# Enigmatisms/cvx_proj

Measured on AMD Instinct MI355X. Metric: local homographies/sec + Mpix/sec warp, 4K pair 200x200 mesh, higher is better.
Workload: dtype f64; 1 GPU; C3: 3840x2160 pair, 2000 correspondences, 200x200 mesh, canvas 4009x2242; mode=pairs, variant=auto, launch=eager, parallelism=pairsx1

## Files before the change

### cvx_proj_amd/_native.py

```python
from __future__ import annotations

import ctypes as C
import os
import sys
from typing import NamedTuple

import numpy as np

_HERE = os.path.dirname(os.path.abspath(__file__))
LIB_PATH = os.environ.get("APAP_HIP_LIB") or os.path.join(_HERE, "libapap_hip.so")

OK, ERR_INVALID_ARG, ERR_NO_DEVICE, ERR_HIP, ERR_SINGULAR, ERR_INDEX, ERR_WORKSPACE = range(7)
ABI_VERSION = 6
PROF_NAMES = ("assemble", "eigen", "invert", "lut", "warp", "eq_hist", "eq_apply", "ransac", "spectral")
PROF_SLOTS = len(PROF_NAMES)
TABLE_STRIDE = 32
DENORM_DOUBLES = 36
VARIANT_AUTO, VARIANT_VALU, VARIANT_MFMA, VARIANT_MFMA4, VARIANT_MFMA4X2 = 0, 1, 2, 3, 4
EIGEN_AUTO, EIGEN_JACOBI, EIGEN_INVERSE_ITERATION = 0, 1, 2
OPT_SOLVER_VARIANT, OPT_EIGEN_SOLVER, OPT_CAREFUL, OPT_PROFILE, OPT_WANT_WAVES, OPT_WARP_ROWS, OPT_WEIGHT_CHUNK_KB, \
    OPT_FUSED_MAX_CELLS, OPT_WARP_FAST, OPT_OVERLAP_PCIE, OPT_PLAN_CELLS, OPT_MOMENTS, OPT_WEIGHTS_F32, \
    OPT_PLAN_SLOTS, OPT_WARP_SAMPLING = range(15)
SAMPLING_NEAREST, SAMPLING_BILINEAR = 0, 1
SAMPLINGS = {"nearest": SAMPLING_NEAREST, "bilinear": SAMPLING_BILINEAR}


class ApapError(RuntimeError):

    def __init__(self, code, message):
        super().__init__(f"[apap_hip error {code}] {message}")
        self.code = code


class ApapSingularError(ApapError, np.linalg.LinAlgError):
    """APAP_ERR_SINGULAR: ``numpy.linalg.inv`` of a cell raised LinAlgError("Singular matrix")
    (apap.py:165-166,203,252)."""


class ApapIndexError(ApapError, IndexError):
    """APAP_ERR_INDEX: ``np.where(i < mesh_h)[0][0]`` found no edge above a canvas index
    (apap.py:207,209)."""


class ApapValueError(ApapError, ValueError):
    """APAP_ERR_INVALID_ARG: what the reference's shape unpacking rejects with ValueError
    (apap.py:129-130,197,199)."""


_ERROR_CLASSES = {ERR_SINGULAR: ApapSingularError, ERR_INDEX: ApapIndexError, ERR_INVALID_ARG: ApapValueError}

STATUS_SINGULAR, STATUS_INDEX, STATUS_UNPREPARED = 1, 2, 4
STATUS_NO_CONVERGENCE = 8
STATUS_MODEL_DEGENERATE = 16
STATUS_MODEL_NO_CONVERGENCE = 32


def raise_for_status(word, who):
    if word & STATUS_SINGULAR:
        raise ApapSingularError(ERR_SINGULAR, f"{who}: Singular matrix")
    if word & STATUS_INDEX:
        raise ApapIndexError(ERR_INDEX, f"{who}: index 0 is out of bounds for axis 0 with size 0 (mesh edges do not cover the canvas)")
    if word & STATUS_UNPREPARED:
        raise ApapValueError(ERR_INVALID_ARG, f"{who}: the warp workspace holds no lookup tables for this mesh / canvas "
                                              "(APAP_WARP_GEOMETRY)")


_f32p = C.POINTER(C.c_float)
_f64p = C.POINTER(C.c_double)
_u8p = C.POINTER(C.c_uint8)
_i32p = C.POINTER(C.c_int)
_i64p = C.POINTER(C.c_longlong)
_vp = C.c_void_p

SIGNATURES = {
    "apap_last_error": (C.c_char_p, []),
    "apap_version": (C.c_char_p, []),
    "apap_abi_version": (C.c_int, []),
    "apap_device_count": (C.c_int, []),
    "apap_ctx_create": (C.c_void_p, []),
    "apap_ctx_destroy": (None, [_vp]),
    "apap_ctx_set_option": (C.c_int, [_vp, C.c_int, C.c_int]),
    "apap_ctx_get_option": (C.c_int, [_vp, C.c_int, _i32p]),
    "apap_ctx_profile_read": (C.c_int, [_vp, _f32p, _i32p]),
    "apap_host_prepare": (C.c_int, [_f32p, _f32p, C.c_int] + [_f32p] * 10),
    "apap_host_dlt_rows": (C.c_int, [_f32p, _f32p, C.c_int, _f32p]),
    "apap_host_prepare_pts": (C.c_int, [_vp, C.c_int, _vp, C.c_int, C.c_int] + [_f32p] * 6 + [_f64p] * 4),
    "apap_host_dlt_rows_pts": (C.c_int, [_f64p, _f64p, C.c_int, C.c_int, _f32p]),
    "apap_host_build_table_rows": (C.c_int, [_f64p, _f32p, C.c_int, _f64p]),
    "apap_host_build_table": (C.c_int, [_f32p, _f32p, _f32p, C.c_int, _f64p]),
    "apap_host_build_table24": (C.c_int, [_f64p, _f32p, C.c_int, _f64p]),
    "apap_host_build_denorm": (C.c_int, [_f32p, _f32p, _f32p, _f32p, _f64p]),
    "apap_local_homography": (C.c_int, [_vp, _f32p, _f32p, C.c_int, _f64p, C.c_int, C.c_int, C.c_double,
                                        C.c_double, _f32p, _f64p, C.c_int]),
    "apap_local_weights": (C.c_int, [_vp, _f32p, C.c_int, _f64p, C.c_int, C.c_double, C.c_double, _f64p, C.c_int]),
    "apap_local_homography_pts": (C.c_int, [_vp, _vp, C.c_int, _vp, C.c_int, C.c_int, _f64p, C.c_int, C.c_int, C.c_double,
                                            C.c_double, _f32p, _f64p, C.c_int]),
    "apap_local_weights_pts": (C.c_int, [_vp, _vp, C.c_int, C.c_int, _f64p, C.c_int, C.c_double, C.c_double, _f64p, C.c_int]),
    "apap_local_warp": (C.c_int, [_vp, _u8p, C.c_int, C.c_int, _f32p, C.c_int, C.c_int, _f64p, C.c_int, _f64p,
                                  C.c_int, C.c_int, C.c_int, C.c_int, C.c_int, _u8p, _f32p, C.c_int]),
    "apap_local_warp_f64": (C.c_int, [_vp, _u8p, C.c_int, C.c_int, _f64p, C.c_int, C.c_int, _f64p, C.c_int, _f64p,
                                      C.c_int, C.c_int, C.c_int, C.c_int, C.c_int, _u8p, _f64p, C.c_int]),
    "apap_local_stitch": (C.c_int, [_vp, _u8p, C.c_int, C.c_int, _u8p, C.c_int, C.c_int, _f32p, C.c_int, C.c_int, _f64p,
                                    C.c_int, _f64p, C.c_int, C.c_int, C.c_int, C.c_int, C.c_int, _u8p, _f32p, C.c_int]),
    "apap_warp_coords": (C.c_int, [_vp, _f32p, C.c_int, C.c_int, _f64p, C.c_int, _f64p, C.c_int, C.c_int, C.c_int,
                                   C.c_int, C.c_int, _f64p, C.c_int]),
    "apap_invert_normalize_flatten": (C.c_int, [_vp, _f32p, C.c_int, _f64p, C.c_int]),
    "apap_uniform_blend": (C.c_int, [_vp, _u8p, _u8p, C.c_int, C.c_int, _u8p, C.c_int]),
    "apap_solve_workspace_bytes": (C.c_size_t, [_vp, C.c_int, C.c_int]),
    "apap_solve_device": (C.c_int, [_vp, _vp, C.c_int, _vp, C.c_int, C.c_double, C.c_double, _vp, _vp, _vp,
                                    C.c_size_t, _vp]),
    "apap_solve_batch_workspace_bytes": (C.c_size_t, [_vp, C.c_int, C.c_int, C.c_int]),
    "apap_solve_batch_device": (C.c_int, [_vp, _vp, C.c_int, _vp, C.c_longlong, C.c_int, C.c_double, C.c_double, _vp, _vp,
                                          C.c_int, _vp, C.c_size_t, _vp]),
    "apap_solve_warp_batch_device": (C.c_int, [_vp, _vp, C.c_int, _vp, C.c_longlong, C.c_double, C.c_double, _vp, _vp, C.c_int, _vp,
                                               C.c_size_t, C.c_int, C.c_int, _vp, C.c_int, _vp, C.c_int, C.c_int, C.c_int, C.c_int,
                                               C.c_int, _vp, C.c_size_t, _vp, _vp]),
    "apap_weights_device": (C.c_int, [_vp, _vp, C.c_int, _vp, C.c_int, C.c_double, C.c_double, _vp, _vp]),
    "apap_warp_workspace_bytes": (C.c_size_t, [C.c_int, C.c_int, C.c_int, C.c_int]),
    "apap_warp_device": (C.c_int, [_vp, _vp, C.c_int, C.c_int, _vp, C.c_int, C.c_int, _vp, C.c_int, _vp, C.c_int,
                                   C.c_int, C.c_int, C.c_int, C.c_int, _vp, _vp, _vp, C.c_size_t, _vp, _vp]),
    "apap_warp_f64_device": (C.c_int, [_vp, _vp, C.c_int, C.c_int, _vp, C.c_int, C.c_int, _vp, C.c_int, _vp, C.c_int,
                                       C.c_int, C.c_int, C.c_int, C.c_int, _vp, _vp, _vp, C.c_size_t, _vp, _vp]),
    "apap_warp_rows_device": (C.c_int, [_vp, _vp, C.c_int, C.c_int, _vp, C.c_int, C.c_int, _vp, C.c_int, _vp, C.c_int,
                                        C.c_int, C.c_int, C.c_int, C.c_int, C.c_int, C.c_int, _vp, _vp, C.c_size_t, _vp,
                                        _vp]),
    "apap_warp_batch_workspace_bytes": (C.c_size_t, [C.c_int, C.c_int, C.c_int, C.c_int, C.c_int]),
    "apap_warp_batch_device": (C.c_int, [_vp, _vp, C.c_longlong, C.c_int, C.c_int, _vp, C.c_longlong, C.c_int, C.c_int, _vp, C.c_int,
                                         C.c_int, _vp, C.c_int, _vp, C.c_int, C.c_int, C.c_int, C.c_int, C.c_int, C.c_int, C.c_int,
                                         _vp, C.c_longlong, _vp, C.c_int, C.c_int, _vp, C.c_size_t, _vp, _vp]),
    "apap_stitch_device": (C.c_int, [_vp, _vp, C.c_int, C.c_int, _vp, C.c_int, C.c_int, _vp, C.c_int, C.c_int, _vp, C.c_int,
                                     _vp, C.c_int, C.c_int, C.c_int, C.c_int, C.c_int, _vp, _vp, _vp, C.c_size_t, _vp, _vp]),
    "apap_warp_coords_device": (C.c_int, [_vp, _vp, C.c_int, C.c_int, _vp, C.c_int, _vp, C.c_int, C.c_int, C.c_int,
                                          C.c_int, C.c_int, _vp, _vp, C.c_size_t, _vp, _vp]),
    "apap_flatten_device": (C.c_int, [_vp, _vp, C.c_int, _vp, _vp, _vp]),
    "apap_blend_device": (C.c_int, [_vp, _vp, _vp, C.c_int, C.c_int, _vp, _vp]),
    "apap_equalize_hist": (C.c_int, [_vp, _u8p, C.c_int, C.c_int, C.c_int, _u8p, C.c_int]),
    "apap_equalize_workspace_bytes": (C.c_size_t, [C.c_int]),
    "apap_equalize_hist_device": (C.c_int, [_vp, _vp, C.c_int, C.c_int, C.c_int, _vp, _vp, C.c_size_t, _vp]),
    "apap_find_homography_ransac": (C.c_int, [_vp, _f32p, _f32p, C.c_int, C.c_double, C.c_int, C.c_ulonglong, _f64p, _u8p,
                                              _i32p, C.c_int]),
    "apap_ransac_workspace_bytes": (C.c_size_t, [C.c_int, C.c_int]),
    "apap_ransac_device": (C.c_int, [_vp, _vp, _vp, C.c_int, C.c_double, C.c_int, C.c_ulonglong, _vp, _vp, _vp, _vp,
                                     C.c_size_t, _vp]),
    "apap_spectral_weights": (C.c_int, [_vp, _f32p, _f32p, _f32p, _f32p, C.c_int, _f64p, _f64p, _f32p, _f32p, _f64p, _f32p,
                                        _f32p, _f64p, C.c_int]),
    "apap_spectral_workspace_bytes": (C.c_size_t, [C.c_int]),
    "apap_spectral_device": (C.c_int, [_vp, _vp, _vp, _vp, _vp, C.c_int, _vp, _f64p, _vp, _vp, _vp, _vp, _vp, _vp, _vp, _vp,
                                       C.c_size_t, _vp]),
    "apap_spectral_affinity": (C.c_int, [_vp, _f32p, _f32p, _f32p, _f32p, C.c_int, _f64p, _f64p, _f64p, C.c_int]),
    "apap_model_solve": (C.c_int, [_vp, _f32p, _f32p, _f32p, C.c_int, _f64p, _f32p, _f64p, C.c_int]),
    "apap_model_workspace_bytes": (C.c_size_t, [C.c_int]),
    "apap_model_solve_device": (C.c_int, [_vp, _vp, _vp, _vp, C.c_int, _f64p, _vp, _vp, _vp, _vp, C.c_size_t, _vp]),
    "apap_spectral_em": (C.c_int, [_vp, _f32p, _f32p, _f32p, _f32p, C.c_int, _f64p, _f64p, _f64p, C.c_int, _f32p, _f32p, _f64p,
                                   _f64p, _f32p, _f32p, _f64p, C.c_int]),
    "apap_spectral_em_device": (C.c_int, [_vp, _vp, _vp, _vp, _vp, C.c_int, _vp, _f64p, _f64p, C.c_int, _vp, _vp, _vp, _vp, _vp, _vp,
                                          _vp, _vp, _vp, C.c_size_t, _vp]),
    "apap_spectral_em_batch_workspace_bytes": (C.c_size_t, [_i32p, C.c_int, _i32p, C.c_int]),
    "apap_spectral_em_batch_device": (C.c_int, [_vp, _vp, _vp, _vp, _vp, _vp, _vp, _i32p, C.c_int, _i32p, _f64p, _f64p, C.c_int,
                                                C.c_int, _vp, _vp, _vp, _vp, _vp, _vp, _vp, _vp, C.c_size_t, _vp]),
    "apap_spectral_em_batch": (C.c_int, [_vp, _f32p, _f32p, _f32p, _f32p, _f64p, _f32p, _i32p, C.c_int, _i32p, _f64p, _f64p,
                                         C.c_int, C.c_int, _f32p, _f64p, _f64p, _f32p, _f32p, _f64p, _i32p, C.c_int]),
    "apap_local_model_workspace_bytes": (C.c_size_t, [C.c_int, C.c_int]),
    "apap_local_model_solve_device": (C.c_int, [_vp, _vp, _vp, _vp, C.c_int, _vp, C.c_int, C.c_double, C.c_double, _f64p, _vp, _vp,
                                                _vp, _vp, C.c_size_t, _vp]),
    "apap_local_model_solve": (C.c_int, [_vp, _f32p, _f32p, _f32p, C.c_int, _f64p, C.c_int, C.c_double, C.c_double, _f64p, _f32p,
                                         _f64p, _i32p, C.c_int]),
    "apap_match_workspace_bytes": (C.c_size_t, [C.c_int, C.c_int]),
    "apap_match_descriptors": (C.c_int, [_vp, _f32p, C.c_int, _f32p, C.c_int, _i32p, _f32p, _i32p, _f32p, C.c_int]),
    "apap_match_descriptors_device": (C.c_int, [_vp, _vp, C.c_int, _vp, C.c_int, _vp, _vp, _vp, _vp, _vp, C.c_size_t, _vp]),
    "apap_match_batch_workspace_bytes": (C.c_size_t, [_i32p, _i32p, C.c_int]),
    "apap_match_descriptors_batch": (C.c_int, [_vp, _f32p, _f32p, _i32p, _i32p, C.c_int, _i32p, _f32p, _i32p, _f32p, C.c_int]),
    "apap_match_descriptors_batch_device": (C.c_int, [_vp, _vp, _vp, _i32p, _i32p, C.c_int, _vp, _vp, _vp, _vp, _vp, C.c_size_t,
                                                      _vp]),
    "apap_sift_window": (C.c_int, [_f32p]),
    "apap_sift_taps": (C.c_int, [_f32p]),
    "apap_sift_workspace_bytes": (C.c_size_t, [C.c_int]),
    "apap_sift_describe": (C.c_int, [_vp, _u8p, C.c_int, C.c_int, C.c_int, _f32p, C.c_int, _f32p, C.c_int]),
    "apap_sift_describe_device": (C.c_int, [_vp, _vp, C.c_int, C.c_int, C.c_int, _vp, C.c_int, _vp, _vp, C.c_size_t, _vp]),
    "apap_sift_describe_batch": (C.c_int, [_vp, C.POINTER(C.c_void_p), _i32p, _i32p, _i32p, C.c_int, _f32p, _i32p, _f32p, C.c_int]),
    "apap_sift_describe_batch_device": (C.c_int, [_vp, C.POINTER(C.c_void_p), _i32p, _i32p, _i32p, C.c_int, _vp, _i32p, _vp, _vp,
                                                  C.c_size_t, _vp]),
    "apap_corner_workspace_bytes": (C.c_size_t, [_i32p, _i32p, C.c_int, C.c_int]),
    "apap_corner_detect": (C.c_int, [_vp, _u8p, C.c_int, C.c_int, C.c_int, C.c_int, C.c_int, C.c_int, _f32p, _i64p, _i32p, C.c_int]),
    "apap_corner_detect_device": (C.c_int, [_vp, _vp, C.c_int, C.c_int, C.c_int, C.c_int, C.c_int, C.c_int, _vp, _vp, _vp, _vp,
                                            C.c_size_t, _vp]),
    "apap_corner_detect_batch": (C.c_int, [_vp, C.POINTER(C.c_void_p), _i32p, _i32p, _i32p, C.c_int, C.c_int, C.c_int, C.c_int, _f32p,
                                           _i64p, _i32p, C.c_int]),
    "apap_corner_detect_batch_device": (C.c_int, [_vp, C.POINTER(C.c_void_p), _i32p, _i32p, _i32p, C.c_int, C.c_int, C.c_int, C.c_int,
                                                  _vp, _vp, _vp, _vp, C.c_size_t, _vp]),
    "apap_image_warp_bounds": (C.c_int, [C.c_int, C.c_int, C.c_int, C.c_int, _f64p, _i32p]),
    "apap_image_warp_workspace_bytes": (C.c_size_t, [C.c_int]),
    "apap_image_warp": (C.c_int, [_vp, _u8p, C.c_int, C.c_int, _u8p, C.c_int, C.c_int, _f64p, C.c_int, C.c_int, C.c_int, C.c_int,
                                  C.c_int, _u8p, C.c_int]),
    "apap_image_warp_device": (C.c_int, [_vp, _vp, C.c_int, C.c_int, _vp, C.c_int, C.c_int, _f64p, C.c_int, C.c_int, C.c_int, C.c_int,
                                         C.c_int, _vp, _vp, C.c_size_t, _vp, _vp]),
    "apap_image_warp_batch": (C.c_int, [_vp, C.POINTER(C.c_void_p), _i32p, _i32p, C.POINTER(C.c_void_p), _i32p, _i32p, _f64p, _i32p,
                                        _i32p, _i32p, _i32p, _i32p, C.c_int, _u8p, _i64p, C.c_int]),
    "apap_image_warp_batch_device": (C.c_int, [_vp, C.POINTER(C.c_void_p), _i32p, _i32p, C.POINTER(C.c_void_p), _i32p, _i32p, _f64p,
                                               _i32p, _i32p, _i32p, _i32p, _i32p, C.c_int, _vp, _i64p, _vp, C.c_size_t, _vp, _vp]),
    "apap_panorama_bounds": (C.c_int, [C.c_int, C.c_int, _i32p, _i32p, _i32p, _i32p, C.c_int, _i32p]),
    "apap_panorama_workspace_bytes": (C.c_size_t, [_i32p, _i32p, _i32p, _i32p, C.c_int]),
    "apap_panorama_mean_of": (C.c_uint, [C.c_uint, C.c_uint]),
    "apap_panorama": (C.c_int, [_vp, _u8p, C.c_int, C.c_int, C.POINTER(C.c_void_p), _i32p, _i32p, C.POINTER(C.c_void_p), _i32p, _i32p,
                                C.POINTER(C.c_void_p), _i32p, C.POINTER(C.c_void_p), _i32p, _i32p, _i32p, _i32p, _i32p, C.c_int, C.c_int,
                                _u8p, _i32p, C.c_int]),
    "apap_panorama_device": (C.c_int, [_vp, _vp, C.c_int, C.c_int, C.POINTER(C.c_void_p), _i32p, _i32p, C.POINTER(C.c_void_p), _i32p,
                                       _i32p, C.POINTER(C.c_void_p), _i32p, C.POINTER(C.c_void_p), _i32p, _i32p, _i32p, _i32p, _i32p,
                                       C.c_int, C.c_int, _vp, _vp, C.c_size_t, _vp, _vp]),
    "apap_panorama_ramp_weight": (C.c_int, [C.c_int, C.c_int, C.c_int, C.c_int, C.c_int]),
    "apap_panorama_ramp_quotients": (None, [C.POINTER(C.c_uint), C.POINTER(C.c_uint), C.c_int, C.POINTER(C.c_uint)]),
}
SIGNATURES["apap_panorama_ramp"] = SIGNATURES["apap_panorama"]
SIGNATURES["apap_panorama_ramp_device"] = SIGNATURES["apap_panorama_device"]
_u64p = C.POINTER(C.c_ulonglong)
_PANO_GEOMETRY = SIGNATURES["apap_panorama"][1][:19]
_PANO_GEOMETRY_DEVICE = SIGNATURES["apap_panorama_device"][1][:19]
SIGNATURES.update({
    "apap_panorama_gain_solve": (C.c_int, [_u64p, _u64p, C.c_int, C.c_double, C.c_double, _f64p, _i32p, _i32p]),
    "apap_panorama_gain_apply": (C.c_int, [_u8p, C.c_int, C.c_int, _u8p]),
    "apap_panorama_gain_stats": (C.c_int, _PANO_GEOMETRY + [C.c_int, _u64p, _u64p, _i32p, C.c_int]),
    "apap_panorama_gain_stats_device": (C.c_int, _PANO_GEOMETRY_DEVICE + [C.c_int, _vp, _vp, _vp, C.c_size_t, _vp, _vp]),
    "apap_panorama_gain": (C.c_int, _PANO_GEOMETRY + [C.c_int, C.c_int, _i32p, _u8p, _i32p, C.c_int]),
    "apap_panorama_gain_device": (C.c_int, _PANO_GEOMETRY_DEVICE + [C.c_int, C.c_int, _i32p, _vp, _vp, C.c_size_t, _vp, _vp]),
    "apap_panorama_auto_gain": (C.c_int, _PANO_GEOMETRY + [C.c_int, C.c_int, C.c_int, C.c_double, C.c_double, _u8p, _u64p, _u64p, _f64p,
                                                           _i32p, _i32p, _i32p, C.c_int]),
    "apap_panorama_auto_gain_device": (C.c_int, _PANO_GEOMETRY_DEVICE + [C.c_int, C.c_int, C.c_int, C.c_double, C.c_double, _vp, _vp, _vp,
                                                                         _vp, _vp, _vp, _vp, C.c_size_t, _vp, _vp]),
})
SIGNATURES.update({
    "apap_box_blur": (C.c_int, [_vp, _u8p, C.c_int, C.c_int, C.c_int, _u8p, C.c_int]),
    "apap_box_blur_device": (C.c_int, [_vp, _vp, C.c_int, C.c_int, C.c_int, _vp, _vp]),
    "apap_panorama_band_workspace_bytes": (C.c_size_t, [C.c_int, C.c_int, _i32p, _i32p, _i32p, _i32p, _i32p, _i32p, C.c_int, C.c_int]),
    "apap_panorama_band": (C.c_int, _PANO_GEOMETRY + [C.c_int, C.c_int, _i32p, _u8p, _i32p, C.c_int]),
    "apap_panorama_band_device": (C.c_int, _PANO_GEOMETRY_DEVICE + [C.c_int, C.c_int, _i32p, _vp, _vp, C.c_size_t, _vp, _vp]),
})

_lib = None
_torch_at_load = False


def lib():
    global _lib, _torch_at_load
    if _lib is None:
        if not os.path.exists(LIB_PATH):
            raise ApapError(ERR_NO_DEVICE, f"{LIB_PATH} not built; run `python -c 'import __graft_entry__ as g; "
                                           "g.build()'` or `make -C cvx_proj_amd/csrc`")
        if "torch" not in sys.modules and os.environ.get("APAP_HIP_PRELOAD_TORCH", "0") == "1":
            try:
                import torch
            except ImportError:
                pass
        _torch_at_load = "torch" in sys.modules
        handle = C.CDLL(LIB_PATH)
        got = handle.apap_abi_version() if hasattr(handle, "apap_abi_version") else 1
        if got != ABI_VERSION:
            raise ApapError(ERR_INVALID_ARG, f"{LIB_PATH} is ABI generation {got}, this binding needs {ABI_VERSION}: rebuild "
                                             "it (make -C cvx_proj_amd/csrc)")
        for name, (res, args) in SIGNATURES.items():
            fn = getattr(handle, name)
            fn.restype = res
            fn.argtypes = args
        _lib = handle
    return _lib


def check(code):
    if code != OK:
        raise _ERROR_CLASSES.get(code, ApapError)(code, lib().apap_last_error().decode("utf-8", "replace"))


class Context:

    def __init__(self, **options):
        self._h = lib().apap_ctx_create()
        if not self._h:
            raise ApapError(ERR_HIP, "apap_ctx_create failed")
        for k, v in options.items():
            self.set(k, v)

    _NAMES = {"variant": OPT_SOLVER_VARIANT, "eigen": OPT_EIGEN_SOLVER, "careful": OPT_CAREFUL, "profile": OPT_PROFILE,
              "want_waves": OPT_WANT_WAVES, "warp_rows": OPT_WARP_ROWS, "weight_chunk_kb": OPT_WEIGHT_CHUNK_KB,
              "fused_max_cells": OPT_FUSED_MAX_CELLS, "warp_fast": OPT_WARP_FAST, "overlap_pcie": OPT_OVERLAP_PCIE,
              "plan_cells": OPT_PLAN_CELLS, "moments": OPT_MOMENTS, "weights_f32": OPT_WEIGHTS_F32,
              "plan_slots": OPT_PLAN_SLOTS, "warp_sampling": OPT_WARP_SAMPLING}

    def set(self, name, value):
        check(lib().apap_ctx_set_option(self._h, self._NAMES[name], int(value)))
        return self

    def get(self, name):
        v = C.c_int(0)
        check(lib().apap_ctx_get_option(self._h, self._NAMES[name], C.byref(v)))
        return v.value

    def profile_read(self):
        ms = (C.c_float * PROF_SLOTS)()
        cnt = (C.c_int * PROF_SLOTS)()
        check(lib().apap_ctx_profile_read(self._h, ms, cnt))
        return {k: (ms[i], cnt[i]) for i, k in enumerate(PROF_NAMES)}

    @property
    def handle(self):
        return self._h

    def close(self):
        if self._h:
            lib().apap_ctx_destroy(self._h)
            self._h = None

    def __del__(self):
        try:
            self.close()
        except Exception:
            pass


def _h(ctx):
    if ctx is None:
        return None
    return C.c_void_p(ctx.handle if isinstance(ctx, Context) else ctx)


def last_error():
    return lib().apap_last_error().decode("utf-8", "replace")


def sampling_value(sampling, who="local_warp"):
    if sampling is None:
        return None
    if not isinstance(sampling, str) or sampling not in SAMPLINGS:
        raise ValueError(f"{who}: sampling must be None, 'nearest' or 'bilinear'; got {sampling!r}")
    return SAMPLINGS[sampling]


class sampling_scope:

    def __init__(self, ctx, sampling, who="local_warp"):
        self._value = sampling_value(sampling, who)
        self._ctx, self._own, self._before = ctx, None, None

    def __enter__(self):
        if self._value is None:
            return self._ctx
        if self._ctx is None:
            self._own = self._ctx = Context()
        before = C.c_int(0)
        check(lib().apap_ctx_get_option(_h(self._ctx), OPT_WARP_SAMPLING, C.byref(before)))
        self._before = before.value
        check(lib().apap_ctx_set_option(_h(self._ctx), OPT_WARP_SAMPLING, self._value))
        return self._ctx

    def __exit__(self, *exc):
        if self._before is not None:
            lib().apap_ctx_set_option(_h(self._ctx), OPT_WARP_SAMPLING, self._before)
        if self._own is not None:
            self._own.close()
        return False


def _ptr(a, ctype):
    return a.ctypes.data_as(C.POINTER(ctype)) if a is not None else None


def as_f32(a, shape_tail=None):
    a = np.ascontiguousarray(a, dtype=np.float32)
    if shape_tail is not None and tuple(a.shape[-len(shape_tail):]) != tuple(shape_tail):
        raise ValueError(f"expected trailing shape {shape_tail}, got {a.shape}")
    return a


def as_points(a):
    a = np.asarray(a)
    a = np.ascontiguousarray(a, dtype=np.float32 if a.dtype == np.float32 else np.float64)
    if a.shape[-1:] != (2,):
        raise ValueError(f"expected trailing shape (2,), got {a.shape}")
    return a, int(a.dtype == np.float64)


def _vptr(a):
    return a.ctypes.data_as(C.c_void_p)


def _ip(a):
    return a.ctypes.data_as(_i32p)


def _dp(a):
    return a.ctypes.data_as(_f64p)


def _addrs(addresses):
    return (C.c_void_p * len(addresses))(*addresses)


def _i32(values):
    return np.array(values, dtype=np.int32)


def _offsets(lengths, name, one, many, rows, max_count, max_rows):
    lengths = [int(x) for x in lengths]
    if not 1 <= len(lengths) <= max_count:
        raise ValueError(f"{name}: {len(lengths)} {many} (1 .. {max_count})")
    if any(not 1 <= x <= max_rows for x in lengths):
        raise ValueError(f"{name}: {one} holds 1 .. 2^{max_rows.bit_length() - 1} {rows}; got {lengths}")
    if sum(lengths) > np.iinfo(np.int32).max:
        raise ValueError(f"{name}: {sum(lengths)} {rows} in all exceed the int32 offsets")
    off = np.zeros(len(lengths) + 1, np.int32)
    off[1:] = np.cumsum(lengths)
    return off


def _image_table(got):
    return (_addrs([a.ctypes.data for a, _ in got]), _i32([a.shape[0] for a, _ in got]), _i32([a.shape[1] for a, _ in got]),
            _i32([c for _, c in got]))


def host_prepare(src, dst):
    src, s64 = as_points(src)
    dst, d64 = as_points(dst)
    if src.shape != dst.shape or src.ndim != 2:
        raise ValueError(f"src/dst must both be (n, 2); got {src.shape} and {dst.shape}")
    n = src.shape[0]
    out = {k: np.empty((3, 3), np.float32) for k in ("N1", "N2", "C1", "C2", "iC2", "iN2")}
    if not s64 and not d64:
        out.update({k: np.empty((n, 2), np.float32) for k in ("nf1", "nf2", "cf1", "cf2")})
        check(lib().apap_host_prepare(_ptr(src, C.c_float), _ptr(dst, C.c_float), n,
                                      *[_ptr(out[k], C.c_float) for k in
                                        ("N1", "N2", "C1", "C2", "iC2", "iN2", "nf1", "nf2", "cf1", "cf2")]))
        return out
    wide = {k: np.empty((n, 2), np.float64) for k in ("nf1", "nf2", "cf1", "cf2")}
    check(lib().apap_host_prepare_pts(_vptr(src), s64, _vptr(dst), d64, n,
                                      *[_ptr(out[k], C.c_float) for k in ("N1", "N2", "C1", "C2", "iC2", "iN2")],
                                      *[_ptr(wide[k], C.c_double) for k in ("nf1", "nf2", "cf1", "cf2")]))
    for k, is64 in (("nf1", s64), ("cf1", s64), ("nf2", d64), ("cf2", d64)):
        out[k] = wide[k] if is64 else wide[k].astype(np.float32)
    return out


def host_dlt_rows(cf1, cf2):
    cf1, a64 = as_points(cf1)
    cf2, b64 = as_points(cf2)
    n = cf1.shape[0]
    aa = np.empty((2 * n, 9), np.float32)
    if not a64 and not b64:
        check(lib().apap_host_dlt_rows(_ptr(cf1, C.c_float), _ptr(cf2, C.c_float), n, _ptr(aa, C.c_float)))
    else:
# ... 909 lines not shown
```

### cvx_proj_amd/csrc/apap_internal.h

```cpp
#pragma once
#include <cstddef>
#include <cstdint>

#include <mutex>
#include <vector>

#include "../../include/apap_hip.h"

namespace apap {

struct ProfSpan {
    int slot;
    void *a, *b;
};

struct DevSlot {
    void *ptr = nullptr;
    size_t cap = 0;
    int dev = -1;
};
enum { S_TABLE, S_VERT, S_DENORM, S_H, S_WORK, S_W, S_IMG, S_OUT, S_MESHW, S_MESHH, S_HINV, S_STATUS, S_AUX, S_COUNT };

}

struct apap_ctx {
    int opt[APAP_OPT_COUNT] = {APAP_VARIANT_AUTO, APAP_EIGEN_AUTO, 1, 0, 4096, 1, 1 << 20, 4096, 1, 0, 0, 30, 0, 0, APAP_SAMPLING_NEAREST};
    std::vector<apap::ProfSpan> spans;
    apap::DevSlot slots[apap::S_COUNT];
    std::mutex mu;
    void *streams[3] = {nullptr, nullptr, nullptr};
    std::vector<void *> events;
    void *pinned = nullptr;
    size_t pinned_cap = 0;
    int pipe_dev = -1;
    int k1_slots[3] = {0, 0, 0};
    int k1_slots_dev = -1;
};

namespace apap {

int opt(const apap_ctx *ctx, int which);

int fail(int code, const char *fmt, ...) __attribute__((format(printf, 2, 3)));

int hip_fail(int hip_error, const char *what);

struct ProfScope {
    ProfScope(apap_ctx *ctx, int slot, void *stream);
    ~ProfScope();
    ProfScope(const ProfScope &) = delete;
    ProfScope &operator=(const ProfScope &) = delete;

  private:
    apap_ctx *ctx_;
    void *stream_, *a_, *b_;
    int slot_;
    bool on_;
};

bool inv3_f64(const double in[9], double out[9]);
bool inv3_f32(const float in[9], float out[9]);

struct SolvePlan {
    int variant;
    int cells_pad;
    int cell_tiles;
    int splits;
    int pts_per_split;
    size_t moment_bytes;
};
SolvePlan plan_solve(int n, int cells, int variant, int batch, int want_waves, int plan_cells = 0, int moments = 30);
int plan_pairs(int cell_tiles, int splits, int batch, int slots);

constexpr int kWarpSetup = APAP_WARP_GEOMETRY | APAP_WARP_CELLS;
constexpr int kWarpRows = APAP_WARP_GATHER;
int warp_phase(apap_ctx *ctx, const uint8_t *d_img, int img_h, int img_w, const uint8_t *d_center, int center_h, int center_w,
               const float *d_Hfwd, int mesh_rows, int mesh_cols, const double *d_mesh_w, int n_w, const double *d_mesh_h,
               int n_h, int final_w, int final_h, int off_x, int off_y, uint8_t *d_out_band, float *d_Hinv_out, void *d_work,
               size_t work_bytes, int *d_status, void *stream, int row_begin, int row_count, int phase, int **d_src_rows);

struct WarpTables {
    const double *hinv_pad;
    const int *lut;
};
WarpTables warp_tables(void *d_work, int mesh_rows, int mesh_cols, int final_w, int final_h);

struct WarpGather {
    const uint8_t *img;
    const uint8_t *center;
    uint8_t *out;
    const double *hinv_pad;
    const int *lut;
    int *status;
    long long img_stride, center_stride, out_stride, hinv_stride;
    int img_h, img_w, center_h, center_w, mesh_rows, mesh_cols, final_w, final_h, off_x, off_y, row_begin, row_count;
};
int warp_bilinear_launch(apap_ctx *ctx, const WarpGather &g, int batch, void *stream);

int panorama_check(int center_h, int center_w, const int *img_h, const int *img_w, const int *mesh_rows, const int *mesh_cols,
                   const int *n_w, const int *n_h, const int *final_w, const int *final_h, const int *off_x, const int *off_y,
                   int n_layers, int mode, const int *ramp, int *bounds, const char *who);
int panorama_device(apap_ctx *ctx, const uint8_t *d_center, int center_h, int center_w, const uint8_t *const *d_imgs, const int *img_h,
                    const int *img_w, const float *const *d_Hfwd, const int *mesh_rows, const int *mesh_cols,
                    const double *const *d_mesh_w, const int *n_w, const double *const *d_mesh_h, const int *n_h, const int *final_w,
                    const int *final_h, const int *off_x, const int *off_y, int n_layers, int mode, const int *ramp, uint8_t *d_out,
                    void *d_work, size_t work_bytes, int *d_status, void *stream, const char *who);

struct PanoGeometry {
    const uint8_t *d_center;
    int center_h, center_w;
    const uint8_t *const *d_imgs;
    const int *img_h, *img_w;
    const float *const *d_Hfwd;
    const int *mesh_rows, *mesh_cols;
    const double *const *d_mesh_w;
    const int *n_w;
    const double *const *d_mesh_h;
    const int *n_h, *final_w, *final_h, *off_x, *off_y;
    int n_layers;
};
enum { kPanoPlain = 0, kPanoGain, kPanoStats, kPanoAuto };
struct PanoJob {
    int what = kPanoPlain;
    int mode = APAP_PANORAMA_MEAN;
    const int *ramp = nullptr;
    const int *band = nullptr;
    uint8_t *d_out = nullptr;
    const int *gain_q = nullptr;
    int step = 1;
    unsigned long long *d_N = nullptr, *d_S = nullptr;
    double sigma_n = 10.0, sigma_g = 0.1;
    double *d_g = nullptr;
    int *d_q = nullptr, *d_flag = nullptr;
};
int panorama_run(apap_ctx *ctx, const PanoGeometry &G, const PanoJob &J, void *d_work, size_t work_bytes, int *d_status, void *stream,
                 const char *who);
int panorama_band_check(int band, const char *who);
int box_blur_check(int h, int w, int radius, const char *who);
int panorama_gain_check(int n_views, const int *step, const int *gain_q, const double *sigma_n, const double *sigma_g, const char *who);
int panorama_gain_solve_host(const unsigned long long *N, const unsigned long long *S, int n_views, double sigma_n, double sigma_g,
                             double *g, int *q);

constexpr int kMoments = 30;

int spectral_run(apap_ctx *ctx, const float *d_src, const float *d_dst, const float *d_c, const float *d_o, int n,
                 const double *d_F, const double *params, const float *d_Hg, const float *d_mask, double *d_segment,
                 float *d_ransac, float *d_original, double *d_info, int *d_status, void *d_work, size_t work_bytes,
                 void *stream, int sync_each);
int spectral_em_run(apap_ctx *ctx, const float *d_src, const float *d_dst, const float *d_c_feats, const float *d_o_feats, int n,
                    const double *d_F, const double *spec_params, const double *model_params, int em_steps, const float *d_mask_in,
                    float *d_H, double *d_info, double *d_segment, float *d_ransac_mask, float *d_original_mask,
                    double *d_spec_info, int *d_status, void *d_work, size_t work_bytes, void *stream, int sync_each);
int spectral_em_batch_run(apap_ctx *ctx, const float *d_src, const float *d_dst, const float *d_c_feats, const float *d_o_feats,
                          const double *d_F, const float *d_mask_in, const int *pair_offset, int n_pairs, const int *pair_of,
                          const double *spec_params, const double *model_params, int n_problems, int em_steps, float *d_H,
                          double *d_info, double *d_segment, float *d_ransac_mask, float *d_original_mask, double *d_spec_info,
                          int *d_status, void *d_work, size_t work_bytes, void *stream, int sync_each);
int spectral_em_batch_check(const int *pair_offset, int n_pairs, const int *pair_of, const double *spec_params,
                            const double *model_params, int n_problems, int em_steps, const char *who);
int local_model_check(int n, int cells, double gamma, double sigma, const double *params, const char *who);
int match_check(const int *q_offset, const int *t_offset, int n_pairs, const char *who);
inline size_t up256(size_t bytes) { return (bytes + 255) / 256 * 256; }

constexpr int kImageMinSide = 7, kImageMaxSide = 32768, kMaxImages = 65535;
inline int image_sides_check(int m, int h, int w, const char *who) {
    if (h < kImageMinSide || h > kImageMaxSide || w < kImageMinSide || w > kImageMaxSide)
        return fail(APAP_ERR_INVALID_ARG, "%s: image %d is %d x %d (sides %d .. %d)", who, m, h, w, kImageMinSide, kImageMaxSide);
    return APAP_OK;
}
inline int image_channels_check(int m, int c, const char *who) {
    if (c != 1 && c != 3) return fail(APAP_ERR_INVALID_ARG, "%s: image %d has %d channels (1 = grey or 3 = BGR)", who, m, c);
    return APAP_OK;
}
int sift_check(const int *heights, const int *widths, const int *channels, int n_images, const int *pt_offset, const char *who);
int corner_check(const int *heights, const int *widths, const int *channels, int n_images, int max_corners, int radius,
                 int quality_permille, const char *who);
int image_warp_check(const int *base_h, const int *base_w, const int *src_h, const int *src_w, const double *M, const int *canvas_w,
                     const int *canvas_h, const int *off_x, const int *off_y, const int *direct_blend, int n_problems,
                     const long long *out_offset, const char *who);
int spectral_affinity_run(const float *d_src, const float *d_dst, const float *d_c, const float *d_o, int n, const double *d_F,
                          const double *params, double *d_M, void *d_work, size_t work_bytes, void *stream);

}

#if defined(__HIP__)
#include <hip/hip_runtime.h>

namespace apap {

// ... 85 lines not shown
```

### cvx_proj_amd/csrc/apap_kernels.hip

```cpp
#include <hip/hip_runtime.h>

#include <cstdlib>
#include <type_traits>
#include <vector>

#include "apap_internal.h"
#include "apap_row_term.h"
#include "apap_warp_dev.h"
#include "apap_weight_dev.h"

namespace {

using apap::inv3;
using apap::rcp_full;

using apap::kMoments;
constexpr int kWave = 64;

struct BatchStride {
    long long table, vertices, moments, denorm, H;
};


constexpr int kExpBits = 9;
constexpr int kExpN = 1 << kExpBits;
constexpr double kExpScale = (double)kExpN * 0x1.71547652b82fep+0;
__constant__ double kExp2Tab[kExpN] = {
    0x1.0000000000000p+0, 0x1.0058c86da1c0ap+0, 0x1.00b1afa5abcbfp+0, 0x1.010ab5b2cbd11p+0,
    0x1.0163da9fb3335p+0, 0x1.01bd1e77170b4p+0, 0x1.02168143b0281p+0, 0x1.027003103b10ep+0,
    0x1.02c9a3e778061p+0, 0x1.032363d42b027p+0, 0x1.037d42e11bbccp+0, 0x1.03d7411915a8ap+0,
    0x1.04315e86e7f85p+0, 0x1.048b9b35659d8p+0, 0x1.04e5f72f654b1p+0, 0x1.0540727fc1762p+0,
    0x1.059b0d3158574p+0, 0x1.05f5c74f0bec2p+0, 0x1.0650a0e3c1f89p+0, 0x1.06ab99fa6407cp+0,
    0x1.0706b29ddf6dep+0, 0x1.0761ead925493p+0, 0x1.07bd42b72a836p+0, 0x1.0818ba42e7d30p+0,
    0x1.0874518759bc8p+0, 0x1.08d0088f8093fp+0, 0x1.092bdf66607e0p+0, 0x1.0987d61701716p+0,
    0x1.09e3ecac6f383p+0, 0x1.0a402331b9715p+0, 0x1.0a9c79b1f3919p+0, 0x1.0af8f03834e52p+0,
    0x1.0b5586cf9890fp+0, 0x1.0bb23d833d93fp+0, 0x1.0c0f145e46c85p+0, 0x1.0c6c0b6bdae53p+0,
    0x1.0cc922b7247f7p+0, 0x1.0d265a4b520bap+0, 0x1.0d83b23395decp+0, 0x1.0de12a7b26300p+0,
    0x1.0e3ec32d3d1a2p+0, 0x1.0e9c7c55189c6p+0, 0x1.0efa55fdfa9c5p+0, 0x1.0f58503328e6dp+0,
    0x1.0fb66affed31bp+0, 0x1.1014a66f951cep+0, 0x1.1073028d7233ep+0, 0x1.10d17f64d9ef1p+0,
    0x1.11301d0125b51p+0, 0x1.118edb6db2dc1p+0, 0x1.11edbab5e2ab6p+0, 0x1.124cbae51a5c8p+0,
    0x1.12abdc06c31ccp+0, 0x1.130b1e264a0e9p+0, 0x1.136a814f204abp+0, 0x1.13ca058cbae1ep+0,
    0x1.1429aaea92de0p+0, 0x1.1489717425438p+0, 0x1.14e95934f312ep+0, 0x1.154962388149ep+0,
    0x1.15a98c8a58e51p+0, 0x1.1609d83606e12p+0, 0x1.166a45471c3c2p+0, 0x1.16cad3c92df73p+0,
    0x1.172b83c7d517bp+0, 0x1.178c554eaea89p+0, 0x1.17ed48695bbc0p+0, 0x1.184e5d23816c9p+0,
    0x1.18af9388c8deap+0, 0x1.1910eba4df41fp+0, 0x1.1972658375d2fp+0, 0x1.19d4013041dc2p+0,
    0x1.1a35beb6fcb75p+0, 0x1.1a979e2363cf8p+0, 0x1.1af99f8138a1cp+0, 0x1.1b5bc2dc40bf0p+0,
    0x1.1bbe084045cd4p+0, 0x1.1c206fb91588fp+0, 0x1.1c82f95281c6bp+0, 0x1.1ce5a51860746p+0,
    0x1.1d4873168b9aap+0, 0x1.1dab6358e15e8p+0, 0x1.1e0e75eb44027p+0, 0x1.1e71aad999e82p+0,
    0x1.1ed5022fcd91dp+0, 0x1.1f387bf9cda38p+0, 0x1.1f9c18438ce4dp+0, 0x1.1fffd7190241ep+0,
    0x1.2063b88628cd6p+0, 0x1.20c7bc96ffc18p+0, 0x1.212be3578a819p+0, 0x1.21902cd3d09b9p+0,
    0x1.21f49917ddc96p+0, 0x1.2259282fc1f27p+0, 0x1.22bdda27912d1p+0, 0x1.2322af0b63bffp+0,
    0x1.2387a6e756238p+0, 0x1.23ecc1c78903ap+0, 0x1.2451ffb82140ap+0, 0x1.24b760c547f15p+0,
    0x1.251ce4fb2a63fp+0, 0x1.25828c65fa1ffp+0, 0x1.25e85711ece75p+0, 0x1.264e450b3cb82p+0,
    0x1.26b4565e27cddp+0, 0x1.271a8b16f0a30p+0, 0x1.2780e341ddf29p+0, 0x1.27e75eeb3ab98p+0,
    0x1.284dfe1f56381p+0, 0x1.28b4c0ea83f36p+0, 0x1.291ba7591bb70p+0, 0x1.2982b17779965p+0,
    0x1.29e9df51fdee1p+0, 0x1.2a5130f50d65cp+0, 0x1.2ab8a66d10f13p+0, 0x1.2b203fc675d1fp+0,
    0x1.2b87fd0dad990p+0, 0x1.2befde4f2e280p+0, 0x1.2c57e39771b2fp+0, 0x1.2cc00cf2f6c18p+0,
    0x1.2d285a6e4030bp+0, 0x1.2d90cc15d5346p+0, 0x1.2df961f641589p+0, 0x1.2e621c1c14833p+0,
    0x1.2ecafa93e2f56p+0, 0x1.2f33fd6a454d2p+0, 0x1.2f9d24abd886bp+0, 0x1.300670653dfe4p+0,
    0x1.306fe0a31b715p+0, 0x1.30d975721b004p+0, 0x1.31432edeeb2fdp+0, 0x1.31ad0cf63eeacp+0,
    0x1.32170fc4cd831p+0, 0x1.3281375752b40p+0, 0x1.32eb83ba8ea32p+0, 0x1.3355f4fb45e20p+0,
    0x1.33c08b26416ffp+0, 0x1.342b46484ebb4p+0, 0x1.3496266e3fa2dp+0, 0x1.35012ba4ea77dp+0,
    0x1.356c55f929ff1p+0, 0x1.35d7a577dd72bp+0, 0x1.36431a2de883bp+0, 0x1.36aeb428335b4p+0,
    0x1.371a7373aa9cbp+0, 0x1.3786581d3f669p+0, 0x1.37f26231e754ap+0, 0x1.385e91be9c811p+0,
    0x1.38cae6d05d866p+0, 0x1.393761742d808p+0, 0x1.39a401b7140efp+0, 0x1.3a10c7a61d55bp+0,
    0x1.3a7db34e59ff7p+0, 0x1.3aeac4bcdf3eap+0, 0x1.3b57fbfec6cf4p+0, 0x1.3bc559212ef89p+0,
    0x1.3c32dc313a8e5p+0, 0x1.3ca0853c10f28p+0, 0x1.3d0e544ede173p+0, 0x1.3d7c4976d27fap+0,
    0x1.3dea64c123422p+0, 0x1.3e58a63b0a09bp+0, 0x1.3ec70df1c5175p+0, 0x1.3f359bf29743fp+0,
    0x1.3fa4504ac801cp+0, 0x1.40132b07a35dfp+0, 0x1.40822c367a024p+0, 0x1.40f153e4a136ap+0,
    0x1.4160a21f72e2ap+0, 0x1.41d016f44d8f5p+0, 0x1.423fb2709468ap+0, 0x1.42af74a1af3f1p+0,
    0x1.431f5d950a897p+0, 0x1.438f6d5817663p+0, 0x1.43ffa3f84b9d4p+0, 0x1.4470018321a1ap+0,
    0x1.44e086061892dp+0, 0x1.4551318eb43ecp+0, 0x1.45c2042a7d232p+0, 0x1.4632fde7006f4p+0,
    0x1.46a41ed1d0057p+0, 0x1.471566f8827d0p+0, 0x1.4786d668b3237p+0, 0x1.47f86d3001fe5p+0,
    0x1.486a2b5c13cd0p+0, 0x1.48dc10fa920a1p+0, 0x1.494e1e192aed2p+0, 0x1.49c052c5916c4p+0,
    0x1.4a32af0d7d3dep+0, 0x1.4aa532feaada6p+0, 0x1.4b17dea6db7d7p+0, 0x1.4b8ab213d5283p+0,
    0x1.4bfdad5362a27p+0, 0x1.4c70d073537cap+0, 0x1.4ce41b817c114p+0, 0x1.4d578e8bb586bp+0,
    0x1.4dcb299fddd0dp+0, 0x1.4e3eeccbd7b2ap+0, 0x1.4eb2d81d8abffp+0, 0x1.4f26eba2e35f0p+0,
    0x1.4f9b2769d2ca7p+0, 0x1.500f8b804f127p+0, 0x1.508417f4531eep+0, 0x1.50f8ccd3deb0dp+0,
    0x1.516daa2cf6642p+0, 0x1.51e2b00da3b14p+0, 0x1.5257de83f4eefp+0, 0x1.52cd359dfd53dp+0,
    0x1.5342b569d4f82p+0, 0x1.53b85df598d78p+0, 0x1.542e2f4f6ad27p+0, 0x1.54a4298571b06p+0,
    0x1.551a4ca5d920fp+0, 0x1.559098bed1bdfp+0, 0x1.56070dde910d2p+0, 0x1.567dac1351819p+0,
    0x1.56f4736b527dap+0, 0x1.576b63f4d854cp+0, 0x1.57e27dbe2c4cfp+0, 0x1.5859c0d59ca07p+0,
    0x1.58d12d497c7fdp+0, 0x1.5948c32824135p+0, 0x1.59c0827ff07ccp+0, 0x1.5a386b5f43d92p+0,
    0x1.5ab07dd485429p+0, 0x1.5b28b9ee20d1ep+0, 0x1.5ba11fba87a03p+0, 0x1.5c19af482fc8fp+0,
    0x1.5c9268a5946b7p+0, 0x1.5d0b4be135accp+0, 0x1.5d84590998b93p+0, 0x1.5dfd902d47c65p+0,
    0x1.5e76f15ad2148p+0, 0x1.5ef07ca0cbf0fp+0, 0x1.5f6a320dceb71p+0, 0x1.5fe411b078d26p+0,
    0x1.605e1b976dc09p+0, 0x1.60d84fd15612ap+0, 0x1.6152ae6cdf6f4p+0, 0x1.61cd3778bc944p+0,
    0x1.6247eb03a5585p+0, 0x1.62c2c91c56acdp+0, 0x1.633dd1d1929fdp+0, 0x1.63b90532205d8p+0,
    0x1.6434634ccc320p+0, 0x1.64afec30678b7p+0, 0x1.652b9febc8fb7p+0, 0x1.65a77e8dcc390p+0,
    0x1.6623882552225p+0, 0x1.669fbcc140be7p+0, 0x1.671c1c70833f6p+0, 0x1.6798a7420a036p+0,
    0x1.68155d44ca973p+0, 0x1.68923e87bfb7ap+0, 0x1.690f4b19e9538p+0, 0x1.698c830a4c8d4p+0,
    0x1.6a09e667f3bcdp+0, 0x1.6a877541ee718p+0, 0x1.6b052fa75173ep+0, 0x1.6b8315a736c75p+0,
    0x1.6c012750bdabfp+0, 0x1.6c7f64b30aa09p+0, 0x1.6cfdcddd47645p+0, 0x1.6d7c62dea2f8ap+0,
    0x1.6dfb23c651a2fp+0, 0x1.6e7a10a38cee8p+0, 0x1.6ef9298593ae5p+0, 0x1.6f786e7ba9fefp+0,
    0x1.6ff7df9519484p+0, 0x1.70777ce1303f6p+0, 0x1.70f7466f42e87p+0, 0x1.71773c4eaa988p+0,
    0x1.71f75e8ec5f74p+0, 0x1.7277ad3ef9011p+0, 0x1.72f8286ead08ap+0, 0x1.7378d02d50b8fp+0,
    0x1.73f9a48a58174p+0, 0x1.747aa5953c849p+0, 0x1.74fbd35d7cbfdp+0, 0x1.757d2df29ce7cp+0,
    0x1.75feb564267c9p+0, 0x1.768069c1a861dp+0, 0x1.77024b1ab6e09p+0, 0x1.7784597eeba8fp+0,
    0x1.780694fde5d3fp+0, 0x1.7888fda749e5dp+0, 0x1.790b938ac1cf6p+0, 0x1.798e56b7fcf03p+0,
    0x1.7a11473eb0187p+0, 0x1.7a94652e958aap+0, 0x1.7b17b0976cfdbp+0, 0x1.7b9b2988fb9ecp+0,
    0x1.7c1ed0130c132p+0, 0x1.7ca2a4456e7a3p+0, 0x1.7d26a62ff86f0p+0, 0x1.7daad5e2850acp+0,
    0x1.7e2f336cf4e62p+0, 0x1.7eb3bedf2e1b9p+0, 0x1.7f3878491c491p+0, 0x1.7fbd5fbab091fp+0,
    0x1.80427543e1a12p+0, 0x1.80c7b8f4abaa9p+0, 0x1.814d2add106d9p+0, 0x1.81d2cb0d1736ap+0,
    0x1.82589994cce13p+0, 0x1.82de968443d9ap+0, 0x1.8364c1eb941f7p+0, 0x1.83eb1bdadb46dp+0,
    0x1.8471a4623c7adp+0, 0x1.84f85b91e07f1p+0, 0x1.857f4179f5b21p+0, 0x1.8606562ab00ecp+0,
    0x1.868d99b4492edp+0, 0x1.87150c27004c2p+0, 0x1.879cad931a436p+0, 0x1.88247e08e1957p+0,
    0x1.88ac7d98a6699p+0, 0x1.8934ac52be8f7p+0, 0x1.89bd0a478580fp+0, 0x1.8a4597875c644p+0,
    0x1.8ace5422aa0dbp+0, 0x1.8b574029db01ep+0, 0x1.8be05bad61778p+0, 0x1.8c69a6bdb5598p+0,
    0x1.8cf3216b5448cp+0, 0x1.8d7ccbc6c19e6p+0, 0x1.8e06a5e0866d9p+0, 0x1.8e90afc931857p+0,
    0x1.8f1ae99157736p+0, 0x1.8fa553499284bp+0, 0x1.902fed0282c8ap+0, 0x1.90bab6ccce12cp+0,
    0x1.9145b0b91ffc6p+0, 0x1.91d0dad829e70p+0, 0x1.925c353aa2fe2p+0, 0x1.92e7bff148396p+0,
    0x1.93737b0cdc5e5p+0, 0x1.93ff669e2802bp+0, 0x1.948b82b5f98e5p+0, 0x1.9517cf65253d1p+0,
    0x1.95a44cbc8520fp+0, 0x1.9630faccf9243p+0, 0x1.96bdd9a7670b3p+0, 0x1.974ae95cba768p+0,
    0x1.97d829fde4e50p+0, 0x1.98659b9bddb5bp+0, 0x1.98f33e47a22a2p+0, 0x1.9981121235681p+0,
    0x1.9a0f170ca07bap+0, 0x1.9a9d4d47f2598p+0, 0x1.9b2bb4d53fe0dp+0, 0x1.9bba4dc5a3dd3p+0,
    0x1.9c49182a3f090p+0, 0x1.9cd81414380f2p+0, 0x1.9d674194bb8d5p+0, 0x1.9df6a0bcfc15ep+0,
    0x1.9e86319e32323p+0, 0x1.9f15f4499c647p+0, 0x1.9fa5e8d07f29ep+0, 0x1.a0360f4424fcbp+0,
    0x1.a0c667b5de565p+0, 0x1.a156f23701b15p+0, 0x1.a1e7aed8eb8bbp+0, 0x1.a2789dacfe68cp+0,
    0x1.a309bec4a2d33p+0, 0x1.a39b1231475f7p+0, 0x1.a42c980460ad8p+0, 0x1.a4be504f696b1p+0,
    0x1.a5503b23e255dp+0, 0x1.a5e25893523d4p+0, 0x1.a674a8af46052p+0, 0x1.a7072b8950a73p+0,
    0x1.a799e1330b358p+0, 0x1.a82cc9be14dcap+0, 0x1.a8bfe53c12e59p+0, 0x1.a95333beb0b7ep+0,
    0x1.a9e6b5579fdbfp+0, 0x1.aa7a6a1897fd2p+0, 0x1.ab0e521356ebap+0, 0x1.aba26d59a09eep+0,
    0x1.ac36bbfd3f37ap+0, 0x1.accb3e100301ep+0, 0x1.ad5ff3a3c2774p+0, 0x1.adf4dcca5a413p+0,
    0x1.ae89f995ad3adp+0, 0x1.af1f4a17a4735p+0, 0x1.afb4ce622f2ffp+0, 0x1.b04a868742ee4p+0,
    0x1.b0e07298db666p+0, 0x1.b17692a8fa8cdp+0, 0x1.b20ce6c9a8952p+0, 0x1.b2a36f0cf3f3ap+0,
    0x1.b33a2b84f15fbp+0, 0x1.b3d11c43bbd62p+0, 0x1.b468415b749b1p+0, 0x1.b4ff9ade433c6p+0,
    0x1.b59728de5593ap+0, 0x1.b62eeb6ddfc87p+0, 0x1.b6c6e29f1c52ap+0, 0x1.b75f0e844bfc6p+0,
    0x1.b7f76f2fb5e47p+0, 0x1.b89004b3a7804p+0, 0x1.b928cf22749e4p+0, 0x1.b9c1ce8e77680p+0,
    0x1.ba5b030a1064ap+0, 0x1.baf46ca7a67a7p+0, 0x1.bb8e0b79a6f1fp+0, 0x1.bc27df9285775p+0,
    0x1.bcc1e904bc1d2p+0, 0x1.bd5c27e2cb5e5p+0, 0x1.bdf69c3f3a207p+0, 0x1.be91462c95b60p+0,
    0x1.bf2c25bd71e09p+0, 0x1.bfc73b0468d30p+0, 0x1.c06286141b33dp+0, 0x1.c0fe06ff301f4p+0,
    0x1.c199bdd85529cp+0, 0x1.c235aab23e61ep+0, 0x1.c2d1cd9fa652cp+0, 0x1.c36e26b34e065p+0,
    0x1.c40ab5fffd07ap+0, 0x1.c4a77b9881650p+0, 0x1.c544778fafb22p+0, 0x1.c5e1a9f8630adp+0,
    0x1.c67f12e57d14bp+0, 0x1.c71cb269e601fp+0, 0x1.c7ba88988c933p+0, 0x1.c8589584661a1p+0,
    0x1.c8f6d9406e7b5p+0, 0x1.c99553dfa8313p+0, 0x1.ca3405751c4dbp+0, 0x1.cad2ee13da7cbp+0,
    0x1.cb720dcef9069p+0, 0x1.cc1164b994d23p+0, 0x1.ccb0f2e6d1675p+0, 0x1.cd50b869d8f0fp+0,
    0x1.cdf0b555dc3fap+0, 0x1.ce90e9be12cb9p+0, 0x1.cf3155b5bab74p+0, 0x1.cfd1f95018d17p+0,
    0x1.d072d4a07897cp+0, 0x1.d113e7ba2c38cp+0, 0x1.d1b532b08c968p+0, 0x1.d256b596f948cp+0,
    0x1.d2f87080d89f2p+0, 0x1.d39a638197a3cp+0, 0x1.d43c8eacaa1d6p+0, 0x1.d4def2158a91fp+0,
    0x1.d5818dcfba487p+0, 0x1.d62461eec14bep+0, 0x1.d6c76e862e6d3p+0, 0x1.d76ab3a99745bp+0,
    0x1.d80e316c98398p+0, 0x1.d8b1e7e2d479dp+0, 0x1.d955d71ff6075p+0, 0x1.d9f9ff37adb4ap+0,
    0x1.da9e603db3285p+0, 0x1.db42fa45c4dfdp+0, 0x1.dbe7cd63a8315p+0, 0x1.dc8cd9ab294e4p+0,
    0x1.dd321f301b460p+0, 0x1.ddd79e065807dp+0, 0x1.de7d5641c0658p+0, 0x1.df2347f63c159p+0,
    0x1.dfc97337b9b5fp+0, 0x1.e06fd81a2ece1p+0, 0x1.e11676b197d17p+0, 0x1.e1bd4f11f8220p+0,
    0x1.e264614f5a129p+0, 0x1.e30bad7dcee90p+0, 0x1.e3b333b16ee12p+0, 0x1.e45af3fe592e8p+0,
    0x1.e502ee78b3ff6p+0, 0x1.e5ab2334ac7eep+0, 0x1.e653924676d76p+0, 0x1.e6fc3bc24e350p+0,
    0x1.e7a51fbc74c83p+0, 0x1.e84e3e4933c7ep+0, 0x1.e8f7977cdb740p+0, 0x1.e9a12b6bc3181p+0,
    0x1.ea4afa2a490dap+0, 0x1.eaf503ccd2be5p+0, 0x1.eb9f4867cca6ep+0, 0x1.ec49c80faa594p+0,
    0x1.ecf482d8e67f1p+0, 0x1.ed9f78d802dc2p+0, 0x1.ee4aaa2188510p+0, 0x1.eef616ca06dd6p+0,
    0x1.efa1bee615a27p+0, 0x1.f04da28a52e59p+0, 0x1.f0f9c1cb6412ap+0, 0x1.f1a61cbdf5be7p+0,
    0x1.f252b376bba97p+0, 0x1.f2ff860a70c22p+0, 0x1.f3ac948dd7274p+0, 0x1.f459df15b82acp+0,
    0x1.f50765b6e4540p+0, 0x1.f5b5288633625p+0, 0x1.f6632798844f8p+0, 0x1.f7116302bd526p+0,
    0x1.f7bfdad9cbe14p+0, 0x1.f86e8f32a4b45p+0, 0x1.f91d802243c89p+0, 0x1.f9ccadbdac61dp+0,
    0x1.fa7c1819e90d8p+0, 0x1.fb2bbf4c0ba54p+0, 0x1.fbdba3692d514p+0, 0x1.fc8bc4866e8adp+0,
    0x1.fd3c22b8f71f1p+0, 0x1.fdecbe15f6314p+0, 0x1.fe9d96b2a23d9p+0, 0x1.ff4eaca4391b6p+0};

__device__ __forceinline__ double exp_neg_scaled(double yu, const double *tab ) {
    constexpr double L = 0x1.62e42fefa39efp-1 / kExpN;
    const int nk = (int)(-yu);
    const double f = __builtin_amdgcn_fract(yu);
    const double t = tab[nk & (kExpN - 1)];
    double p = fma(f, L * L * L * L / 24, -(L * L * L / 6));
    p = fma(f, p, L * L / 2);
    p = fma(f, p, -L);
    p = fma(f, p, 1.0);
    return __builtin_ldexp(t * p, nk >> kExpBits);
}

__device__ __forceinline__ double cell_weight_sq_of(double x, double scaled_inv_sigma2, double gamma2, const double *tab) {
    const double y = __builtin_amdgcn_rsq(x);
    double g = x * y;
    const double e = fma(-g, y, 1.0);
    const double c = fma(e, 0.375, 0.5);
    g = fma(g * e, c, g);
    return fmax(exp_neg_scaled(g * scaled_inv_sigma2, tab), gamma2);
}
__device__ __forceinline__ double cell_weight_sq_tab(double vx, double vy, double sx, double sy,
                                                     double scaled_inv_sigma2, double gamma2, const double *tab) {
    const double dx = vx - sx;
    const double dy = vy - sy;
    return cell_weight_sq_of(fma(dx, dx, fma(dy, dy, 1e-300)), scaled_inv_sigma2, gamma2, tab);
}
__device__ __forceinline__ double cell_weight_sq_row(double vx, double sx, double row_term,
                                                     double scaled_inv_sigma2, double gamma2, const double *tab) {
    const double dx = vx - sx;
    return cell_weight_sq_of(fma(dx, dx, row_term), scaled_inv_sigma2, gamma2, tab);
}

__device__ __forceinline__ double cell_weight_sq_f32(float vx, float vy, float2 s, float neg_scale, float gamma2) {
    const float dx = vx - s.x;
    const float dy = vy - s.y;
    const float d = __builtin_amdgcn_sqrtf(__builtin_fmaf(dx, dx, dy * dy));
    return (double)fmaxf(__builtin_amdgcn_exp2f(d * neg_scale), gamma2);
}

constexpr double kGammaCutF64 = 0x1p128;
__host__ __device__ inline double k1_gamma2(double gamma, bool w32) {
    if (gamma >= (w32 ? 1.0 : kGammaCutF64)) return 1.0;
    return gamma > 0.0 ? gamma * gamma : 0.0;
}

constexpr double kTraceFloorF64 = 1e-280;
constexpr double kTraceFloorW32 = 0x1p-40;

constexpr long long kTable24Marker = 0x7ff8242424242424ll;
__device__ __forceinline__ bool table_is_24(const double *__restrict__ table) {
    return __double_as_longlong(table[28]) == kTable24Marker;
}

typedef double double4_t __attribute__((ext_vector_type(4)));
constexpr int kChunk = 64;
static_assert(kChunk % 16 == 0 && kChunk % 4 == 0, "chunk must split evenly over 256 threads and 4-keypoint steps");

struct K1Block {
    int p_begin, p_end, nchunks;
    __device__ __forceinline__ K1Block(const double *__restrict__ &table, const double *__restrict__ &vertices,
                                       const BatchStride &bs, int n, int split, int pts_per_split) {
        table += (long long)blockIdx.z * bs.table;
        vertices += (long long)blockIdx.z * bs.vertices;
        p_begin = min(n, split * pts_per_split);
        p_end = min(n, p_begin + pts_per_split);
        nchunks = (p_end - p_begin + kChunk - 1) / kChunk;
    }
};

__device__ __forceinline__ double2 cell_vertex(const double *__restrict__ vertices, int cell, int cells) {
    const int cc = min(cell, cells - 1);
    return make_double2(vertices[2 * cc], vertices[2 * cc + 1]);
}

template <int kThreads>
__device__ __forceinline__ void exp_table_copy(double *s_exp2, int tid) {
    for (int j = tid; j < kExpN; j += kThreads) s_exp2[j] = kExp2Tab[j];
}
template <int kThreads>
struct ExpTableStage {
    static_assert(kExpN % kThreads == 0 || kThreads % kExpN == 0, "exp table vs block size");
    static constexpr int kPerThread = (kExpN + kThreads - 1) / kThreads;
    double v[kPerThread];
    __device__ __forceinline__ void fetch(int tid) {
#pragma unroll
        for (int i = 0; i < kPerThread; ++i) v[i] = kExp2Tab[(tid + i * kThreads) & (kExpN - 1)];
    }
    __device__ __forceinline__ void publish(double *s_exp2, int tid) const {
#pragma unroll
        for (int i = 0; i < kPerThread; ++i) s_exp2[(tid + i * kThreads) & (kExpN - 1)] = v[i];
    }
};

__host__ __device__ constexpr int lds_off(int r, int c) { return r * 256 + ((c ^ ((r & 1) << 4)) << 3); }
#define APAP_LDS_PIECE_OFF(r, slot) ((r) * 256 + ((slot) ^ (((r) & 1) << 3)) * 16)
constexpr bool lds_swizzles_agree() {
    for (int r = 0; r < 2; ++r)
        for (int slot = 0; slot < 16; ++slot)
            if (APAP_LDS_PIECE_OFF(r, slot) != lds_off(r, 2 * slot) || APAP_LDS_PIECE_OFF(r, slot) + 8 != lds_off(r, 2 * slot + 1))
                return false;
    return true;
}
static_assert(lds_swizzles_agree(), "a staged piece lands where lds_off looks for its two columns, for both row parities");

template <int kThreads>
using ChunkStage = double2[kChunk * 16 / kThreads];
template <int kThreads>
__device__ __forceinline__ void chunk_load(ChunkStage<kThreads> &stage, const double *__restrict__ table, int tid, int first_row,
                                           int end_row) {
#pragma unroll
    for (int i = 0; i < kChunk * 16 / kThreads; ++i) {
        const int q = tid + kThreads * i;
        const int p = first_row + (q >> 4);
        stage[i] = (p < end_row) ? *reinterpret_cast<const double2 *>(table + (size_t)p * APAP_TABLE_STRIDE + 2 * (q & 15))
                                 : make_double2(0.0, 0.0);
    }
}
#define APAP_CHUNK_STORE(kThreads, buf, stage, tid)                                          \
    do {                                                                                     \
        _Pragma("unroll") for (int i_ = 0; i_ < kChunk * 16 / (kThreads); ++i_) {            \
            const int q_ = (tid) + (kThreads) * i_;                                          \
            const int r_ = q_ >> 4, slot_ = q_ & 15;                                         \
            *reinterpret_cast<double2 *>(&(buf)[APAP_LDS_PIECE_OFF(r_, slot_)]) = (stage)[i_]; \
        }                                                                                    \
    } while (0)

constexpr int kBufferWord3 = 0x00020000;
constexpr int kTableRowBytes = APAP_TABLE_STRIDE * 8;
static_assert(kTableRowBytes == 256, "an LDS row is a table row");
struct ChunkWindow {
    __amdgpu_buffer_rsrc_t rsrc;
    __device__ __forceinline__ ChunkWindow(const double *__restrict__ table, int first_row, int end_row) {
        const int rows = min(kChunk, end_row - first_row);
        rsrc = __builtin_amdgcn_make_buffer_rsrc(const_cast<double *>(table) + (size_t)first_row * APAP_TABLE_STRIDE, 0,
                                                 rows * kTableRowBytes, kBufferWord3);
    }
    __device__ __forceinline__ double2 load16(int lane_off) const {
        typedef unsigned int u32x4 __attribute__((ext_vector_type(4)));
        const u32x4 v = __builtin_amdgcn_raw_buffer_load_b128(rsrc, lane_off, 0, 0);
        return make_double2(__longlong_as_double(((long long)v[1] << 32) | v[0]), __longlong_as_double(((long long)v[3] << 32) | v[2]));
    }
    __device__ __forceinline__ double load8(int lane_off) const {
        typedef unsigned int u32x2 __attribute__((ext_vector_type(2)));
        const u32x2 v = __builtin_amdgcn_raw_buffer_load_b64(rsrc, lane_off, 0, 0);
        return __longlong_as_double(((long long)v[1] << 32) | v[0]);
    }
};
constexpr bool lds_pieces_are_4096_apart() {
    for (int t = 0; t < 256; ++t)
        for (int i = 0; i < 4; ++i)
            if (APAP_LDS_PIECE_OFF((t + 256 * i) >> 4, (t + 256 * i) & 15) != APAP_LDS_PIECE_OFF(t >> 4, t & 15) + 4096 * i) return false;
    return true;
}
static_assert(lds_pieces_are_4096_apart(), "a thread's four pieces: one LDS address and four immediates");

template <bool kW32>
struct CellWeight {
    static constexpr int kXyColumn = kW32 ? 29 : 30;
    using Xy = std::conditional_t<kW32, float2, double2>;
    double vx, vy, scaled_inv_sigma2, gamma2;
    float vxf, vyf, neg_scale_f, gamma2f;
    const double *exp2;
    __device__ __forceinline__ void set(double2 v, double inv_sigma2, double gamma2_, const double *s_exp2) {
        vx = v.x, vy = v.y;
        scaled_inv_sigma2 = inv_sigma2 * kExpScale;
        gamma2 = gamma2_;
        vxf = (float)vx, vyf = (float)vy;
        neg_scale_f = (float)(inv_sigma2 * -0x1.71547652b82fep+0), gamma2f = (float)gamma2;
        exp2 = s_exp2;
    }
    static __device__ __forceinline__ Xy read(const unsigned char *at) { return *reinterpret_cast<const Xy *>(at); }
    __device__ __forceinline__ double sq(Xy s) const {
        if constexpr (kW32) return cell_weight_sq_f32(vxf, vyf, s, neg_scale_f, gamma2f);
        else return cell_weight_sq_tab(vx, vy, s.x, s.y, scaled_inv_sigma2, gamma2, exp2);
    }
    __device__ __forceinline__ double sq(const unsigned char *at) const { return sq(read(at)); }
    __device__ __forceinline__ double sq_row(double sx, double row_term) const {
        return cell_weight_sq_row(vx, sx, row_term, scaled_inv_sigma2, gamma2, exp2);
    }
};

template <bool kM24>
struct Sums16 {
    double4_t acc0 = {0.0, 0.0, 0.0, 0.0}, acc1 = {0.0, 0.0, 0.0, 0.0};
    double acc_a = 0.0, acc_b = 0.0;
    __device__ __forceinline__ void step(double w2, const unsigned char *at0, const unsigned char *at1) {
        const double b0 = *reinterpret_cast<const double *>(at0);
        const double b1 = *reinterpret_cast<const double *>(at1);
        acc0 = __builtin_amdgcn_mfma_f64_16x16x4f64(w2, b0, acc0, 0, 0, 0);
        if constexpr (kM24) {
            acc_a = __builtin_amdgcn_mfma_f64_4x4x4f64(w2, b1, acc_a, 0, 0, 0);
            acc_b = __builtin_amdgcn_mfma_f64_4x4x4f64(w2, *reinterpret_cast<const double *>(at1 + 32), acc_b, 0, 0, 0);
        } else {
            acc1 = __builtin_amdgcn_mfma_f64_16x16x4f64(w2, b1, acc1, 0, 0, 0);
        }
    }
    __device__ __forceinline__ void step(double w2, double b0, double b1, double b1b) {
        acc0 = __builtin_amdgcn_mfma_f64_16x16x4f64(w2, b0, acc0, 0, 0, 0);
        if constexpr (kM24) {
            acc_a = __builtin_amdgcn_mfma_f64_4x4x4f64(w2, b1, acc_a, 0, 0, 0);
            acc_b = __builtin_amdgcn_mfma_f64_4x4x4f64(w2, b1b, acc_b, 0, 0, 0);
        } else {
            acc1 = __builtin_amdgcn_mfma_f64_16x16x4f64(w2, b1, acc1, 0, 0, 0);
        }
    }
};

struct K1Pairs {
    int pairs, splits, tiles;
};
__host__ __device__ inline void k1_unit(const K1Pairs &pp, int i, int &tile, int &split, bool &paired) {
    const int base = pp.pairs / pp.splits, rem = pp.pairs % pp.splits;
    paired = i < pp.pairs;
    if (paired) {
        split = i % pp.splits;
        tile = 2 * (i / pp.splits);
        return;
    }
    int k = i - pp.pairs;
    const int n1 = pp.tiles - 2 * (base + 1), n0 = pp.tiles - 2 * base;
    if (k < rem * n1) {
        split = k / n1;
        tile = 2 * (base + 1) + k % n1;
    } else {
        k -= rem * n1;
        split = rem + k / n0;
        tile = 2 * base + k % n0;
    }
}

__host__ __device__ constexpr int d16_cell(int lane, int i) { return (lane >> 4) + 4 * i; }
__host__ __device__ constexpr int d16_column(int lane) { return lane & 15; }
__host__ __device__ constexpr int d4_cell(int lane) { return 4 * ((lane >> 2) & 3) + (lane >> 4); }
__host__ __device__ constexpr int d4_column(int lane) { return lane & 3; }

constexpr int kLinePitch = 144;
constexpr int kLineStageBytes = 32 * kLinePitch;
__host__ __device__ constexpr int line_stage_off(int column, int cell) { return column * kLinePitch + cell * 8; }
__host__ __device__ constexpr int line_column(int lane, int j) { return 8 * j + (lane >> 3); }
__host__ __device__ constexpr int line_cell(int lane) { return 2 * (lane & 7); }
__host__ __device__ constexpr int line_stores(int sums) { return (sums + 7) / 8; }
template <int kSums>
constexpr bool line_layout_covers() {
    static_assert(kSums == 30 || kSums == 24, "the two tables");
    int staged[32][16] = {}, stored[32][16] = {};
    for (int lane = 0; lane < 64; ++lane) {
        for (int i = 0; i < 4; ++i) {
            ++staged[d16_column(lane)][d16_cell(lane, i)];
            if (kSums == 30) ++staged[16 + d16_column(lane)][d16_cell(lane, i)];
        }
        if (kSums == 24) {
            ++staged[16 + d4_column(lane)][d4_cell(lane)];
            ++staged[20 + d4_column(lane)][d4_cell(lane)];
        }
        for (int j = 0; j < line_stores(kSums); ++j) {
            const int c = line_column(lane, j);
            if (c >= 32 || line_cell(lane) + 1 >= 16 || line_stage_off(c, line_cell(lane)) % 16 != 0 ||
                line_stage_off(c, line_cell(lane) + 1) != line_stage_off(c, line_cell(lane)) + 8)
                return false;
            if (c < kSums) ++stored[c][line_cell(lane)], ++stored[c][line_cell(lane) + 1];
        }
    }
    for (int c = 0; c < 32; ++c)
        for (int cell = 0; cell < 16; ++cell)
            if (staged[c][cell] != (c < (kSums == 30 ? 32 : 24)) || stored[c][cell] != (c < kSums)) return false;
    return true;
}
static_assert(line_layout_covers<30>() && line_layout_covers<24>(),
              "the line layout stores every sum of a 16-cell group once, columns from kSums on never, from what the D layouts staged");
static_assert(kLinePitch % 16 == 0 && 16 * 8 <= kLinePitch && 4 * kLineStageBytes <= 2 * kChunk * 256,
              "16-byte reads of whole rows; four waves' stages fit the two chunk buffers");

typedef double double2_t __attribute__((ext_vector_type(2)));
__device__ __forceinline__ void slab_store_line(double *p, double2_t v) {
    asm volatile("global_store_dwordx4 %0, %1, off sc1\n\ts_nop 1" ::"v"(p), "v"(v) : "memory");
}

__global__ __launch_bounds__(256) void k_assemble_valu(const double *__restrict__ table, int n,
                                                       const double *__restrict__ vertices, int cells,
                                                       int cells_pad, double gamma2, double inv_sigma2,
                                                       int pts_per_split, double *__restrict__ moments,
                                                       BatchStride bs) {
    __shared__ double s_exp2[kExpN];
    exp_table_copy<256>(s_exp2, threadIdx.x);
    __syncthreads();
    table += (long long)blockIdx.z * bs.table;
    vertices += (long long)blockIdx.z * bs.vertices;
    moments += (long long)blockIdx.z * bs.moments;
    const int lane = threadIdx.x & 63;
    const int wave = __builtin_amdgcn_readfirstlane(threadIdx.x >> 6);
    const int cell = (blockIdx.x * 4 + wave) * kWave + lane;
    if (cell - lane >= cells_pad) return;
    const double2 v = cell_vertex(vertices, cell, cells);
    const double vx = v.x, vy = v.y;
    const int p0 = min(n, (int)blockIdx.y * pts_per_split);
    const int p1 = min(n, p0 + pts_per_split);
    const double scaled_inv_sigma2 = inv_sigma2 * kExpScale;

    double acc[kMoments];
#pragma unroll
    for (int j = 0; j < kMoments; ++j) acc[j] = 0.0;

    double sx = 0.0, sy = 0.0;
    if (p0 < p1) {
        sx = table[(size_t)p0 * APAP_TABLE_STRIDE + 30];
        sy = table[(size_t)p0 * APAP_TABLE_STRIDE + 31];
    }
    __builtin_amdgcn_s_waitcnt(0x0070);
    for (int p = p0; p < p1; ++p) {
        const double *__restrict__ row = table + (size_t)p * APAP_TABLE_STRIDE;
        const double *__restrict__ nxt = table + (size_t)min(p + 1, p1 - 1) * APAP_TABLE_STRIDE;
        const double nsx = nxt[30], nsy = nxt[31];
        double r[kMoments];
#pragma unroll
        for (int j = 0; j < kMoments; ++j) r[j] = row[j];
        __builtin_amdgcn_sched_barrier(0);
        const double w2 = cell_weight_sq_tab(vx, vy, sx, sy, scaled_inv_sigma2, gamma2, s_exp2);
#pragma unroll
        for (int j = 0; j < kMoments; ++j) acc[j] = fma(w2, r[j], acc[j]);
        __builtin_amdgcn_sched_barrier(0);
        sx = nsx;
        sy = nsy;
    }
    double *dst = moments + (size_t)blockIdx.y * kMoments * cells_pad + cell;
#pragma unroll
    for (int j = 0; j < kMoments; ++j) dst[(size_t)j * cells_pad] = acc[j];
}

template <int kWaves, bool kM24, bool kW32, int kGroups, bool kLevel>
__device__ __forceinline__ void k1_mfma_tiles(unsigned char (&lds)[2][kChunk * 256], double *s_exp2, double (&s_row)[2][kChunk][2],
                                              const double *__restrict__ table, const double *__restrict__ vertices, int cells,
                                              int cells_pad, double gamma2, double inv_sigma2, double *__restrict__ slab, int tile,
                                              const K1Block &blk) {
    constexpr int kThreads = kWaves * 64;
    const int tid = threadIdx.x;
    ExpTableStage<kThreads> exp_stage;
    exp_stage.fetch(tid);
    const int lane = tid & 63;
    const int wave = tid >> 6;
    const int kgrp = lane >> 4;
    const int col = lane & 15;
    CellWeight<kW32> weight[kGroups];
#pragma unroll
    for (int t = 0; t < kGroups; ++t)
        weight[t].set(cell_vertex(vertices, (tile + t) * (16 * kWaves) + wave * 16 + col, cells), inv_sigma2, gamma2, s_exp2);
    const int p_begin = blk.p_begin, p_end = blk.p_end, nchunks = blk.nchunks;

    constexpr bool kCanShare = !kW32;
    bool share = false;
    double row_v = 0.0;
    bool row_owner = false;
    int off_row[kGroups];
    if constexpr (kCanShare) {
        static_assert(kWaves == 4 && kThreads >= apap::kRowOwners && kChunk == apap::kRowChunk, "the side table's owners");
        const int first = tile * (16 * kWaves);
        auto uniform_bits = [](double v) {
            const long long b = __double_as_longlong(v);
            return (long long)(((unsigned long long)(unsigned)__builtin_amdgcn_readfirstlane((int)(b >> 32)) << 32) |
                               (unsigned)__builtin_amdgcn_readfirstlane((int)b));
        };
        const long long a_bits = uniform_bits(cell_vertex(vertices, first, cells).y);
        long long seen[kGroups];
#pragma unroll
        for (int t = 0; t < kGroups; ++t) seen[t] = __double_as_longlong(cell_vertex(vertices, first + 64 * t + lane, cells).y);
        long long b_bits = a_bits;
#pragma unroll
        for (int t = kGroups - 1; t >= 0; --t) {
            const unsigned long long other = __ballot(seen[t] != a_bits);
            const int l = other ? __builtin_ctzll(other) : 0;
            const long long there = (long long)(((unsigned long long)(unsigned)__builtin_amdgcn_readlane((int)(seen[t] >> 32), l) << 32) |
                                                (unsigned)__builtin_amdgcn_readlane((int)seen[t], l));
            b_bits = other ? there : b_bits;
        }
        bool mine = true;
#pragma unroll
        for (int t = 0; t < kGroups; ++t) mine = mine && apap::row_is_shared(seen[t], a_bits, b_bits);
        share = __all(mine);
        const int wave_r = __builtin_amdgcn_readfirstlane(wave);
        row_owner = wave_r < apap::kRowOwners / 64;
        row_v = __longlong_as_double(apap::row_owner_value(wave_r * 64) == 0 ? a_bits : b_bits);
#pragma unroll
        for (int t = 0; t < kGroups; ++t)
            off_row[t] = apap::row_read_off(0, 0, kgrp, apap::row_value(__double_as_longlong(weight[t].vy), a_bits));
    }
    static_assert(kThreads == 256, "four pieces a thread, 16 rows apart");
    const int piece_src = (tid >> 4) * kTableRowBytes + (tid & 15) * 16;
    const int piece_dst = APAP_LDS_PIECE_OFF(tid >> 4, tid & 15);
    const int row_src = apap::row_owner_keypoint(tid) * kTableRowBytes + 31 * 8;
    auto window_load = [&](ChunkStage<kThreads> &to, const ChunkWindow &win) {
#pragma unroll
        for (int i = 0; i < 4; ++i) to[i] = win.load16(piece_src + 4096 * i);
    };
    auto window_store = [&](unsigned char *buf, const ChunkStage<kThreads> &from) {
#pragma unroll
        for (int i = 0; i < 4; ++i) *reinterpret_cast<double2 *>(buf + piece_dst + 4096 * i) = from[i];
    };
    auto row_fetch = [&](const ChunkWindow &win) { return win.load8(row_src); };
    auto row_publish = [&](int buffer, double sy) {
        const double dy = row_v - sy;
        s_row[buffer][apap::row_owner_keypoint(tid)][apap::row_owner_value(tid)] = fma(dy, dy, 1e-300);
    };

    ChunkStage<kThreads> stage;
    const int off_xy = lds_off(kgrp, CellWeight<kW32>::kXyColumn), off_b0 = lds_off(kgrp, col);
    const int off_b1 = lds_off(kgrp, 16 + (kM24 ? (lane & 3) : col));
    Sums16<kM24> sums[kGroups];
    auto step2 = [&](const double (&w2)[kGroups], const unsigned char *at0, const unsigned char *at1) {
        const double b0 = *reinterpret_cast<const double *>(at0);
        const double b1 = *reinterpret_cast<const double *>(at1);
        const double b1b = kM24 ? *reinterpret_cast<const double *>(at1 + 32) : 0.0;
#pragma unroll
        for (int t = 0; t < kGroups; ++t) sums[t].step(w2[t], b0, b1, b1b);
    };
    const ChunkWindow first_window(table, p_begin, p_end);
    if (nchunks > 0) window_load(stage, first_window);
    double row_y0 = 0.0;
    if constexpr (kCanShare) {
        if (row_owner && nchunks > 0) row_y0 = row_fetch(first_window);
    }
    exp_stage.publish(s_exp2, tid);
    if (nchunks > 0) window_store(lds[0], stage);
    if constexpr (kCanShare) {
        if (row_owner && nchunks > 0) row_publish(0, row_y0);
    }
    __syncthreads();
    __builtin_amdgcn_s_waitcnt(0x0070);
    const int nfull = (p_end - p_begin) / kChunk;
    auto chunks = [&](auto row_tag) {
        constexpr bool kRow = decltype(row_tag)::value;
        auto w2_row = [&](int t, double sx, const unsigned char *rbuf, int s) {
            return weight[t].sq_row(sx, *reinterpret_cast<const double *>(rbuf + off_row[t] + apap::kRowStepBytes * s));
        };
        for (int c = 0; c < nfull; ++c) {
            if constexpr (kLevel) {
                if (4 * c < nfull) __builtin_amdgcn_s_setprio(3);
                else if (4 * c < 2 * nfull) __builtin_amdgcn_s_setprio(2);
                else if (4 * c < 3 * nfull) __builtin_amdgcn_s_setprio(1);
                else __builtin_amdgcn_s_setprio(0);
            }
            ChunkStage<kThreads> next;
            double row_y = 0.0;
            {
                const int next_row = p_begin + (c + 1) * kChunk;
                const ChunkWindow window(table, next_row, c + 1 < nchunks ? p_end : next_row);
                window_load(next, window);
                if constexpr (kRow) {
                    if (row_owner) row_y = row_fetch(window);
                }
            }
            const unsigned char *buf = lds[c & 1];
            const unsigned char *rbuf = reinterpret_cast<const unsigned char *>(s_row[c & 1]);
            if constexpr (kGroups == 1) {
#pragma unroll
                for (int s0 = 0; s0 < kChunk / 4; s0 += 8) {
                    double w2[8];
#pragma unroll
                    for (int g = 0; g < 8; ++g) {
                        if constexpr (kRow) w2[g] = w2_row(0, *reinterpret_cast<const double *>(buf + off_xy + 1024 * (s0 + g)), rbuf, s0 + g);
                        else w2[g] = weight[0].sq(buf + off_xy + 1024 * (s0 + g));
                    }
                    __builtin_amdgcn_sched_barrier(0);
#pragma unroll
                    for (int g = 0; g < 8; ++g) sums[0].step(w2[g], buf + off_b0 + 1024 * (s0 + g), buf + off_b1 + 1024 * (s0 + g));
                    __builtin_amdgcn_sched_barrier(0);
                }
            } else {
                constexpr int kSteps = kW32 ? 2 : 4;
#pragma unroll
                for (int s0 = 0; s0 < kChunk / 4; s0 += kSteps) {
                    double w2[kSteps][kGroups];
#pragma unroll
                    for (int g = 0; g < kSteps; ++g) {
                        if constexpr (kRow) {
                            const double sx = *reinterpret_cast<const double *>(buf + off_xy + 1024 * (s0 + g));
#pragma unroll
                            for (int t = 0; t < kGroups; ++t) w2[g][t] = w2_row(t, sx, rbuf, s0 + g);
                        } else {
                            const auto xy = CellWeight<kW32>::read(buf + off_xy + 1024 * (s0 + g));
#pragma unroll
                            for (int t = 0; t < kGroups; ++t) w2[g][t] = weight[t].sq(xy);
                        }
                    }
                    __builtin_amdgcn_sched_barrier(0);
#pragma unroll
                    for (int g = 0; g < kSteps; ++g) step2(w2[g], buf + off_b0 + 1024 * (s0 + g), buf + off_b1 + 1024 * (s0 + g));
                    __builtin_amdgcn_sched_barrier(0);
                }
            }
            window_store(lds[(c + 1) & 1], next);
            if constexpr (kRow) {
                if (row_owner) row_publish((c + 1) & 1, row_y);
            }
            __syncthreads();
        }
        if (nfull < nchunks) {
            const unsigned char *buf = lds[nfull & 1];
            const unsigned char *rbuf = reinterpret_cast<const unsigned char *>(s_row[nfull & 1]);
            const int steps_here = (p_end - p_begin - nfull * kChunk + 3) >> 2;
            for (int s1 = 0; s1 < steps_here; ++s1) {
                if constexpr (kGroups == 1) {
                    double w2;
                    if constexpr (kRow) w2 = w2_row(0, *reinterpret_cast<const double *>(buf + off_xy + 1024 * s1), rbuf, s1);
                    else w2 = weight[0].sq(buf + off_xy + 1024 * s1);
                    sums[0].step(w2, buf + off_b0 + 1024 * s1, buf + off_b1 + 1024 * s1);
                } else {
                    double w2[kGroups];
                    if constexpr (kRow) {
                        const double sx = *reinterpret_cast<const double *>(buf + off_xy + 1024 * s1);
#pragma unroll
                        for (int t = 0; t < kGroups; ++t) w2[t] = w2_row(t, sx, rbuf, s1);
                    } else {
                        const auto xy = CellWeight<kW32>::read(buf + off_xy + 1024 * s1);
#pragma unroll
                        for (int t = 0; t < kGroups; ++t) w2[t] = weight[t].sq(xy);
                    }
                    step2(w2, buf + off_b0 + 1024 * s1, buf + off_b1 + 1024 * s1);
                }
            }
            __syncthreads();
        }
    };
    if constexpr (kCanShare) {
        if (share) chunks(std::true_type{});
        else chunks(std::false_type{});
    } else {
        chunks(std::false_type{});
    }

    static_assert(kWaves * kLineStageBytes <= (int)sizeof(lds), "a stage per wave");
    constexpr int kSums = kM24 ? 24 : kMoments;
    const int wave_u = __builtin_amdgcn_readfirstlane(wave);
    unsigned char *stage_lds = &lds[0][0] + wave_u * kLineStageBytes;
#pragma unroll
    for (int t = 0; t < kGroups; ++t) {
        const int cell_base = (tile + t) * (16 * kWaves) + wave_u * 16;
        if (t > 0) {
            __builtin_amdgcn_fence(__ATOMIC_RELEASE, "wavefront");
            __builtin_amdgcn_wave_barrier();
            __builtin_amdgcn_fence(__ATOMIC_ACQUIRE, "wavefront");
        }
#pragma unroll
        for (int i = 0; i < 4; ++i) {
            *reinterpret_cast<double *>(stage_lds + line_stage_off(d16_column(lane), d16_cell(lane, i))) = sums[t].acc0[i];
            if constexpr (!kM24)
                *reinterpret_cast<double *>(stage_lds + line_stage_off(16 + d16_column(lane), d16_cell(lane, i))) = sums[t].acc1[i];
        }
        if constexpr (kM24) {
            *reinterpret_cast<double *>(stage_lds + line_stage_off(16 + d4_column(lane), d4_cell(lane))) = sums[t].acc_a;
            *reinterpret_cast<double *>(stage_lds + line_stage_off(20 + d4_column(lane), d4_cell(lane))) = sums[t].acc_b;
        }
        __builtin_amdgcn_fence(__ATOMIC_RELEASE, "wavefront");
        __builtin_amdgcn_wave_barrier();
        __builtin_amdgcn_fence(__ATOMIC_ACQUIRE, "wavefront");
        if (cell_base < cells_pad) {
#pragma unroll
            for (int j = 0; j < line_stores(kSums); ++j) {
                const int c = line_column(lane, j);
                const double2_t v = *reinterpret_cast<const double2_t *>(stage_lds + line_stage_off(c, line_cell(lane)));
                if (c < kSums) slab_store_line(slab + (size_t)c * cells_pad + cell_base + line_cell(lane), v);
            }
        }
    }
}

template <int kWaves, bool kM24, bool kW32>
__global__ __launch_bounds__(kWaves * 64) void k_assemble_mfma(const double *__restrict__ table, int n,
                                                       const double *__restrict__ vertices, int cells,
                                                       int cells_pad, double gamma2, double inv_sigma2,
                                                       int pts_per_split, double *__restrict__ moments,
                                                       BatchStride bs, K1Pairs pp) {
    __shared__ __attribute__((aligned(16))) unsigned char lds[2][kChunk * 256];
    __shared__ double s_exp2[kExpN];
    __shared__ __attribute__((aligned(16))) double s_row[2][kChunk][2];
    int tile = blockIdx.x, split = blockIdx.y;
    bool paired = false;
    if (pp.pairs > 0) k1_unit(pp, (int)blockIdx.x, tile, split, paired);
    const K1Block blk(table, vertices, bs, n, split, pts_per_split);
    constexpr int kSums = kM24 ? 24 : kMoments;
    double *slab = moments + (long long)blockIdx.z * bs.moments + (size_t)split * kSums * cells_pad;
    if (paired)
        k1_mfma_tiles<kWaves, kM24, kW32, 2, true>(lds, s_exp2, s_row, table, vertices, cells, cells_pad, gamma2, inv_sigma2, slab, tile, blk);
    else if (pp.pairs > 0)
        k1_mfma_tiles<kWaves, kM24, kW32, 1, true>(lds, s_exp2, s_row, table, vertices, cells, cells_pad, gamma2, inv_sigma2, slab, tile, blk);
    else
        k1_mfma_tiles<kWaves, kM24, kW32, 1, false>(lds, s_exp2, s_row, table, vertices, cells, cells_pad, gamma2, inv_sigma2, slab, tile, blk);
}

template <int kGroups, int kQuads, bool kW32>
__global__ __launch_bounds__(256) void k_assemble_mfma4(const double *__restrict__ table, int n,
                                                        const double *__restrict__ vertices, int cells,
                                                        int cells_pad, double gamma2, double inv_sigma2,
                                                        int pts_per_split, double *__restrict__ moments,
                                                        BatchStride bs) {
    __shared__ __attribute__((aligned(16))) unsigned char lds[2][kChunk * 256];
    const K1Block blk(table, vertices, bs, n, (int)blockIdx.y, pts_per_split);
    moments += (long long)blockIdx.z * bs.moments;
    __shared__ double s_exp2[kExpN];
    exp_table_copy<256>(s_exp2, threadIdx.x);
    const int tid = threadIdx.x;
    const int lane = tid & 63;
    const int wave = tid >> 6;
    const int kgrp = lane >> 4;
    const int col = lane & 15;
    const int cell0 = (blockIdx.x * 4 + wave) * (16 * kGroups);
    CellWeight<kW32> weight[kGroups];
#pragma unroll
    for (int g = 0; g < kGroups; ++g) weight[g].set(cell_vertex(vertices, cell0 + 16 * g + col, cells), inv_sigma2, gamma2, s_exp2);
    const int p_begin = blk.p_begin, p_end = blk.p_end, nchunks = blk.nchunks;

    ChunkStage<256> stage;
    const int off_xy = lds_off(kgrp, CellWeight<kW32>::kXyColumn);
    const int off_lo = lds_off(kgrp, lane & 3), off_hi = lds_off(kgrp, 16 + (lane & 3));
    double acc[kGroups][kQuads];
#pragma unroll
    for (int g = 0; g < kGroups; ++g)
#pragma unroll
        for (int m = 0; m < kQuads; ++m) acc[g][m] = 0.0;
    if (nchunks > 0) {
        chunk_load<256>(stage, table, tid, p_begin, p_end);
        APAP_CHUNK_STORE(256, lds[0], stage, tid);
    }
    __syncthreads();
    __builtin_amdgcn_s_waitcnt(0x0070);
    for (int c = 0; c < nchunks; ++c) {
        if (c + 1 < nchunks) chunk_load<256>(stage, table, tid, p_begin + (c + 1) * kChunk, p_end);
        const unsigned char *buf = lds[c & 1];
#pragma unroll
        for (int s = 0; s < kChunk / 4; ++s) {
            double bv[kQuads];
#pragma unroll
            for (int m = 0; m < kQuads; ++m)
                bv[m] = *reinterpret_cast<const double *>(buf + (m < 4 ? off_lo : off_hi) + 32 * (m & 3) + 1024 * s);
            double w2[kGroups];
            const auto xy = CellWeight<kW32>::read(buf + off_xy + 1024 * s);
#pragma unroll
            for (int g = 0; g < kGroups; ++g) w2[g] = weight[g].sq(xy);
#pragma unroll
            for (int m = 0; m < kQuads; ++m)
#pragma unroll
                for (int g = 0; g < kGroups; ++g)
                    acc[g][m] = __builtin_amdgcn_mfma_f64_4x4x4f64(w2[g], bv[m], acc[g][m], 0, 0, 0);
        }
        if (c + 1 < nchunks) APAP_CHUNK_STORE(256, lds[(c + 1) & 1], stage, tid);
        __syncthreads();
    }
    constexpr int kSums = kQuads == 6 ? 24 : kMoments;
    double *slab = moments + (size_t)blockIdx.y * kSums * cells_pad;
    const int dcell = d4_cell(lane);
    const int dj = d4_column(lane);
#pragma unroll
    for (int g = 0; g < kGroups; ++g) {
        const int ci = cell0 + 16 * g + dcell;
        if (ci < cells_pad) {
#pragma unroll
            for (int m = 0; m < kQuads; ++m)
                if (4 * m + dj < kSums) slab[(size_t)(4 * m + dj) * cells_pad + ci] = acc[g][m];
        }
    }
}

__host__ __device__ constexpr int tri(int i, int j) {
    return i <= j ? i * (19 - i) / 2 + (j - i) : j * (19 - j) / 2 + (i - j);
}

template <int P, int Q>
__device__ __forceinline__ void jacobi_rotate(double (&a)[45], double (&v)[81]) {
    const double apq = a[tri(P, Q)];
    const double app = a[tri(P, P)];
    const double aqq = a[tri(Q, Q)];
    const double theta = 0.5 * (aqq - app) / apq;
    double t = copysign(1.0, theta) / (fabs(theta) + sqrt(fma(theta, theta, 1.0)));
    t = (apq != 0.0) ? t : 0.0;
    const double c = 1.0 / sqrt(fma(t, t, 1.0));
    const double s = t * c;
    a[tri(P, P)] = fma(-t, apq, app);
    a[tri(Q, Q)] = fma(t, apq, aqq);
    a[tri(P, Q)] = 0.0;
#pragma unroll
    for (int k = 0; k < 9; ++k) {
        if (k != P && k != Q) {
            const double akp = a[tri(k, P)];
            const double akq = a[tri(k, Q)];
            a[tri(k, P)] = fma(c, akp, -(s * akq));
            a[tri(k, Q)] = fma(s, akp, c * akq);
        }
    }
#pragma unroll
    for (int k = 0; k < 9; ++k) {
        const double vkp = v[9 * k + P];
        const double vkq = v[9 * k + Q];
        v[9 * k + P] = fma(c, vkp, -(s * vkq));
        v[9 * k + Q] = fma(s, vkp, c * vkq);
    }
}

__device__ __forceinline__ void jacobi_sweep(double (&a)[45], double (&v)[81]) {
#define APAP_ROW(p, q) jacobi_rotate<p, q>(a, v);
    APAP_ROW(0, 1) APAP_ROW(0, 2) APAP_ROW(0, 3) APAP_ROW(0, 4) APAP_ROW(0, 5) APAP_ROW(0, 6) APAP_ROW(0, 7) APAP_ROW(0, 8)
    APAP_ROW(1, 2) APAP_ROW(1, 3) APAP_ROW(1, 4) APAP_ROW(1, 5) APAP_ROW(1, 6) APAP_ROW(1, 7) APAP_ROW(1, 8)
    APAP_ROW(2, 3) APAP_ROW(2, 4) APAP_ROW(2, 5) APAP_ROW(2, 6) APAP_ROW(2, 7) APAP_ROW(2, 8)
    APAP_ROW(3, 4) APAP_ROW(3, 5) APAP_ROW(3, 6) APAP_ROW(3, 7) APAP_ROW(3, 8)
    APAP_ROW(4, 5) APAP_ROW(4, 6) APAP_ROW(4, 7) APAP_ROW(4, 8)
    APAP_ROW(5, 6) APAP_ROW(5, 7) APAP_ROW(5, 8)
    APAP_ROW(6, 7) APAP_ROW(6, 8)
    APAP_ROW(7, 8)
#undef APAP_ROW
}

__device__ __forceinline__ void mul3(const double *x, const double *y, double *out) {
#pragma unroll
    for (int i = 0; i < 3; ++i)
#pragma unroll
        for (int j = 0; j < 3; ++j)
            out[3 * i + j] = fma(x[3 * i + 2], y[6 + j], fma(x[3 * i + 1], y[3 + j], x[3 * i] * y[j]));
}

constexpr int kMaxSweeps = 15;

__device__ __forceinline__ double jacobi_eigvec(double (&a)[45], int pick_rank, double (&h)[9]) {
    double v[81];
#pragma unroll
    for (int k = 0; k < 81; ++k) v[k] = (k % 10 == 0) ? 1.0 : 0.0;
    for (int sweep = 0; sweep < kMaxSweeps; ++sweep) {
        jacobi_sweep(a, v);
        double off2 = 0.0, trace = 0.0;
#pragma unroll
        for (int i = 0; i < 9; ++i) {
            trace += fabs(a[tri(i, i)]);
#pragma unroll
            for (int j = i + 1; j < 9; ++j) off2 = fma(a[tri(i, j)], a[tri(i, j)], off2);
        }
        const bool done = off2 <= 1e-34 * trace * trace;
        if (__all(done)) break;
    }
    int best = 0;
    double lam0 = 0.0, lam1 = 0.0;
#pragma unroll
    for (int i = 0; i < 9; ++i) {
// ... 1170 lines not shown
#pragma unroll
                for (int t = 0; t < kRows; ++t)
#pragma unroll
                    for (int k = 0; k < 4; ++k) off[t][k] = (idx == t * 4 + k) ? o : off[t][k];
            }
        }
    }
#pragma unroll
    for (int t = 0; t < kRows; ++t)
#pragma unroll
        for (int k = 0; k < 4; ++k) px[t][k] = gather_px(img, off[t][k], last);
    const int y_store_end = ready ? y_end : y_first;
#pragma unroll
    for (int t = 0; t < kRows; ++t) {
        const int y = y_first + t;
        if (y >= y_store_end) break;
        if (kBlend) {
#pragma unroll
            for (int k = 0; k < 4; ++k)
                px[t][k] = blend_center(px[t][k], center, y - off_y, j0 + k - off_x, center_h, center_w, clast);
        }
        APAP_STORE_PX4(out + ((size_t)(y - row_begin) * (size_t)final_w) * 3 + (unsigned)j0 * 3u, px[t], npx);
    }
}

__global__ __launch_bounds__(256) void k_warp_coords(const double *__restrict__ hinv_pad, int mesh_cols,
                                                     const int *__restrict__ lut, int final_w,
                                                     int final_h, int off_x, int off_y,
                                                     double *__restrict__ coords) {
    const size_t total = (size_t)final_w * final_h;
    const size_t g = (size_t)blockIdx.x * blockDim.x + threadIdx.x;
    if (g >= total) return;
    const int i = (int)(g / final_w);
    const int j = (int)(g - (size_t)i * final_w);
    const int cell = lut[i] * mesh_cols + lut[final_h + j];
    double tx, ty;
    target_of(hinv_pad, cell, (double)(j - off_x), (double)(i - off_y), tx, ty);
    coords[2 * g] = tx;
    coords[2 * g + 1] = ty;
}

__global__ __launch_bounds__(256) void k_flatten(const float *__restrict__ H, int cells,
                                                 double *__restrict__ out, int *status) {
    const int cell = blockIdx.x * blockDim.x + threadIdx.x;
    if (cell >= cells) return;
    double m[9], r[9];
#pragma unroll
    for (int k = 0; k < 9; ++k) m[k] = (double)H[(size_t)cell * 9 + k];
    if (!inv3(m, r)) atomicOr(status, APAP_STATUS_SINGULAR);
    float f[9];
#pragma unroll
    for (int k = 0; k < 9; ++k) f[k] = (float)r[k];
    const float d = f[8];
#pragma unroll
    for (int k = 0; k < 9; ++k) f[k] = f[k] / d;
#pragma unroll
    for (int rr = 0; rr < 3; ++rr)
#pragma unroll
        for (int c = 0; c < 3; ++c) out[(size_t)cell * 9 + 3 * c + rr] = (double)f[3 * rr + c];
}

__global__ __launch_bounds__(256) void k_blend(const uint8_t *__restrict__ a, const uint8_t *__restrict__ b,
                                               size_t pixels, uint8_t *__restrict__ out) {
    for (size_t p = (size_t)blockIdx.x * blockDim.x + threadIdx.x; p < pixels;
         p += (size_t)gridDim.x * blockDim.x) {
        const uint8_t *pa = a + 3 * p, *pb = b + 3 * p;
        const unsigned a0 = pa[0], a1 = pa[1], a2 = pa[2], b0 = pb[0], b1 = pb[1], b2 = pb[2];
        const bool both = (a0 + a1 + a2 > 0) && (b0 + b1 + b2 > 0);
        const unsigned sh = both ? 1u : 0u;
        out[3 * p] = (uint8_t)((a0 + b0) >> sh);
        out[3 * p + 1] = (uint8_t)((a1 + b1) >> sh);
        out[3 * p + 2] = (uint8_t)((a2 + b2) >> sh);
    }
}

inline int hip_fail(hipError_t e, const char *what) { return apap::hip_fail((int)e, what); }
using apap::ProfScope;

}

namespace apap {

int hip_fail(int hip_error, const char *what) {
    return fail(APAP_ERR_HIP, "%s: %s", what, hipGetErrorString((hipError_t)hip_error));
}

int opt(const apap_ctx *ctx, int which) {
    static const apap_ctx defaults;
    return (ctx ? ctx : &defaults)->opt[which];
}

ProfScope::ProfScope(apap_ctx *ctx, int slot, void *stream)
    : ctx_(ctx), stream_(stream), a_(nullptr), b_(nullptr), slot_(slot), on_(ctx && ctx->opt[APAP_OPT_PROFILE]) {
    if (!on_) return;
    hipEvent_t a, b;
    on_ = hipEventCreate(&a) == hipSuccess && hipEventCreate(&b) == hipSuccess;
    if (!on_) return;
    a_ = a;
    b_ = b;
    (void)hipEventRecord(a, (hipStream_t)stream_);
}

ProfScope::~ProfScope() {
    if (!on_) return;
    (void)hipEventRecord((hipEvent_t)b_, (hipStream_t)stream_);
    ctx_->spans.push_back(ProfSpan{slot_, a_, b_});
}

SolvePlan plan_solve(int n, int cells, int variant, int batch, int want_waves, int plan_cells, int moments) {
    SolvePlan p{};
    if (variant == APAP_VARIANT_AUTO) variant = APAP_VARIANT_MFMA;
    p.variant = variant;
    p.cell_tiles = (cells + kWave - 1) / kWave;
    p.cells_pad = p.cell_tiles * kWave;
    int splits = 1;
    if (want_waves < 1) want_waves = 4096;
    const int waves_per_2tiles = variant == APAP_VARIANT_MFMA || variant == APAP_VARIANT_MFMA4 ? 8
                                 : variant == APAP_VARIANT_MFMA4X2 ? 4 : 2;
    const long long plan_tiles = plan_cells > 0 ? (plan_cells + kWave - 1) / kWave : (long long)p.cell_tiles * batch;
    while (splits < 32 && plan_tiles * waves_per_2tiles * splits < 2 * want_waves && n / (splits * 2) >= kChunk) splits *= 2;
    int pps = (n + splits - 1) / splits;
    pps = (pps + kChunk - 1) / kChunk * kChunk;
    p.splits = (n + pps - 1) / pps;
    p.pts_per_split = pps;
    p.moment_bytes = (size_t)p.splits * (moments == 24 ? 24 : kMoments) * p.cells_pad * sizeof(double);
    return p;
}

int plan_pairs(int cell_tiles, int splits, int batch, int slots) {
    const long long units = (long long)cell_tiles * splits;
    if (batch != 1 || slots < 1 || units <= slots || units >= 2ll * slots) return 0;
    const long long room = (long long)splits * (cell_tiles / 2);
    return (int)(units - slots < room ? units - slots : room);
}

}

extern "C" {

apap_ctx *apap_ctx_create(void) { return new (std::nothrow) apap_ctx; }

void apap_ctx_destroy(apap_ctx *ctx) {
    if (!ctx) return;
    for (apap::ProfSpan &sp : ctx->spans) {
        (void)hipEventDestroy((hipEvent_t)sp.a);
        (void)hipEventDestroy((hipEvent_t)sp.b);
    }
    for (apap::DevSlot &sl : ctx->slots)
        if (sl.ptr) (void)hipFree(sl.ptr);
    for (void *e : ctx->events) (void)hipEventDestroy((hipEvent_t)e);
    for (void *st : ctx->streams)
        if (st) (void)hipStreamDestroy((hipStream_t)st);
    if (ctx->pinned) (void)hipHostFree(ctx->pinned);
    delete ctx;
}

int apap_ctx_set_option(apap_ctx *ctx, int option, int value) {
    if (!ctx) return apap::fail(APAP_ERR_INVALID_ARG, "apap_ctx_set_option: null context (NULL means the defaults and cannot be changed)");
    bool ok = false;
    switch (option) {
        case APAP_OPT_SOLVER_VARIANT: ok = value >= APAP_VARIANT_AUTO && value <= APAP_VARIANT_MFMA4X2; break;
        case APAP_OPT_EIGEN_SOLVER: ok = value >= APAP_EIGEN_AUTO && value <= APAP_EIGEN_INVERSE_ITERATION; break;
        case APAP_OPT_CAREFUL:
        case APAP_OPT_PROFILE: ok = value == 0 || value == 1; break;
        case APAP_OPT_WANT_WAVES: ok = value >= 1; break;
        case APAP_OPT_WARP_ROWS: ok = value == 0 || value == 1 || value == 2 || value == 4 || value == 5 || value == 6 || value == 8; break;
        case APAP_OPT_WEIGHT_CHUNK_KB: ok = value >= 1; break;
        case APAP_OPT_FUSED_MAX_CELLS:
        case APAP_OPT_PLAN_CELLS:
        case APAP_OPT_PLAN_SLOTS: ok = value >= 0; break;
        case APAP_OPT_WARP_FAST:
        case APAP_OPT_OVERLAP_PCIE:
        case APAP_OPT_WEIGHTS_F32: ok = value == 0 || value == 1; break;
        case APAP_OPT_MOMENTS: ok = value == 30 || value == 24; break;
        case APAP_OPT_WARP_SAMPLING: ok = value == APAP_SAMPLING_NEAREST || value == APAP_SAMPLING_BILINEAR; break;
        default: return apap::fail(APAP_ERR_INVALID_ARG, "apap_ctx_set_option: unknown option %d", option);
    }
    if (!ok) return apap::fail(APAP_ERR_INVALID_ARG, "apap_ctx_set_option: value %d is not valid for option %d", value, option);
    ctx->opt[option] = value;
    return APAP_OK;
}

int apap_ctx_get_option(const apap_ctx *ctx, int option, int *value) {
    if (!value || option < 0 || option >= APAP_OPT_COUNT) return apap::fail(APAP_ERR_INVALID_ARG, "apap_ctx_get_option: bad argument");
    *value = apap::opt(ctx, option);
    return APAP_OK;
}

int apap_ctx_profile_read(apap_ctx *ctx, float *ms, int *launches) {
    if (!ctx || !ms || !launches) return apap::fail(APAP_ERR_INVALID_ARG, "apap_ctx_profile_read: null argument");
    for (int k = 0; k < APAP_PROF_SLOTS; ++k) {
        ms[k] = 0.0f;
        launches[k] = 0;
    }
    int rc = APAP_OK;
    for (apap::ProfSpan &sp : ctx->spans) {
        float t = 0.0f;
        hipError_t e = hipEventSynchronize((hipEvent_t)sp.b);
        if (e == hipSuccess) e = hipEventElapsedTime(&t, (hipEvent_t)sp.a, (hipEvent_t)sp.b);
        if (e != hipSuccess) rc = hip_fail(e, "apap_ctx_profile_read");
        ms[sp.slot] += t;
        launches[sp.slot] += 1;
        (void)hipEventDestroy((hipEvent_t)sp.a);
        (void)hipEventDestroy((hipEvent_t)sp.b);
    }
    ctx->spans.clear();
    return rc;
}

size_t apap_solve_batch_workspace_bytes(apap_ctx *ctx, int n, int cells, int batch) {
    if (n < 1 || cells < 1 || batch < 1) return 0;
    return apap::plan_solve(n, cells, apap::opt(ctx, APAP_OPT_SOLVER_VARIANT), batch, apap::opt(ctx, APAP_OPT_WANT_WAVES), apap::opt(ctx, APAP_OPT_PLAN_CELLS),
                            apap::opt(ctx, APAP_OPT_MOMENTS)).moment_bytes * (size_t)batch;
}

size_t apap_solve_workspace_bytes(apap_ctx *ctx, int n, int cells) { return apap_solve_batch_workspace_bytes(ctx, n, cells, 1); }

}

static int solve_batch_impl(apap_ctx *ctx, const double *d_tables, int n, const double *d_vertices, long long vertices_stride,
                            int cells, double gamma, double sigma, const double *d_denorms, float *d_H,
                            int batch, void *d_work, size_t work_bytes, void *stream, const WarpEmit &we) {
    if (!d_tables || !d_vertices || !d_denorms || !d_H || !d_work)
        return apap::fail(APAP_ERR_INVALID_ARG, "apap_solve_device: null device pointer");
    if (n < 1 || cells < 1 || batch < 1 || batch > 65535 || vertices_stride < 0)
        return apap::fail(APAP_ERR_INVALID_ARG, "apap_solve_device: n=%d cells=%d batch=%d", n, cells, batch);
    const bool m24 = apap::opt(ctx, APAP_OPT_MOMENTS) == 24;
    const bool w32 = m24 && apap::opt(ctx, APAP_OPT_WEIGHTS_F32) != 0;
    if (m24 && apap::opt(ctx, APAP_OPT_SOLVER_VARIANT) == APAP_VARIANT_VALU)
        return apap::fail(APAP_ERR_INVALID_ARG, "apap_solve_device: APAP_OPT_MOMENTS = 24 has no VALU form (use AUTO, MFMA, MFMA4 or MFMA4X2)");
    const apap::SolvePlan p = apap::plan_solve(n, cells, apap::opt(ctx, APAP_OPT_SOLVER_VARIANT), batch, apap::opt(ctx, APAP_OPT_WANT_WAVES),
                                               apap::opt(ctx, APAP_OPT_PLAN_CELLS), m24 ? 24 : 30);
    if (work_bytes < p.moment_bytes * (size_t)batch)
        return apap::fail(APAP_ERR_WORKSPACE, "apap_solve_device: workspace %zu < %zu bytes", work_bytes,
                          p.moment_bytes * (size_t)batch);
    hipStream_t s = (hipStream_t)stream;
    const double inv_sigma = 1.0 / (sigma * sigma);
    const double inv_sigma2 = 2.0 * inv_sigma;
    const double gamma2 = k1_gamma2(gamma, w32);
    const double trace_floor = w32 ? kTraceFloorW32 : kTraceFloorF64;
    double *moments = (double *)d_work;
    BatchStride bs;
    bs.table = (long long)n * APAP_TABLE_STRIDE;
    bs.vertices = vertices_stride;
    bs.moments = (long long)(p.moment_bytes / sizeof(double));
    bs.denorm = APAP_DENORM_DOUBLES;
    bs.H = (long long)cells * 9;
    const int pick_rank = 9 - (2 * n < 9 ? 2 * n : 9);
    const int careful = apap::opt(ctx, APAP_OPT_CAREFUL);
    const int plan_cells = apap::opt(ctx, APAP_OPT_PLAN_CELLS);
    if (!m24 && apap::opt(ctx, APAP_OPT_SOLVER_VARIANT) == APAP_VARIANT_AUTO &&
        (plan_cells > 0 ? (long long)plan_cells : (long long)cells * batch) <= apap::opt(ctx, APAP_OPT_FUSED_MAX_CELLS)) {
        ProfScope prof(ctx, APAP_PROF_ASSEMBLE, s);
        const dim3 grid((cells + 15) / 16, 1, batch);
        if (apap::opt(ctx, APAP_OPT_EIGEN_SOLVER) == APAP_EIGEN_JACOBI)
            hipLaunchKernelGGL(k_solve_small<false>, grid, dim3(kSmallThreads), 0, s, d_tables, n, d_vertices, cells, gamma, inv_sigma,
                               d_denorms, pick_rank, careful, d_H, bs, we);
        else
            hipLaunchKernelGGL(k_solve_small<true>, grid, dim3(kSmallThreads), 0, s, d_tables, n, d_vertices, cells, gamma, inv_sigma,
                               d_denorms, pick_rank, careful, d_H, bs, we);
        const hipError_t e = hipGetLastError();
        if (e != hipSuccess) return hip_fail(e, "apap_solve_device launch");
        return APAP_OK;
    }
    {
        ProfScope prof(ctx, APAP_PROF_ASSEMBLE, s);
        using K1 = void (*)(const double *, int, const double *, int, int, double, double, int, double *, BatchStride);
        static const struct {
            K1 form[3];
            int tiles;
        } k1[] = {
            {{k_assemble_valu, nullptr, nullptr}, 4},
            {{nullptr, nullptr, nullptr}, 1},
            {{k_assemble_mfma4<1, 8, false>, k_assemble_mfma4<1, 6, false>, k_assemble_mfma4<1, 6, true>}, 1},
            {{k_assemble_mfma4<2, 8, false>, k_assemble_mfma4<2, 6, false>, k_assemble_mfma4<2, 6, true>}, 2},
        };
        using K1Mfma = void (*)(const double *, int, const double *, int, int, double, double, int, double *, BatchStride, K1Pairs);
        static const K1Mfma k1_mfma[3] = {k_assemble_mfma<4, false, false>, k_assemble_mfma<4, true, false>, k_assemble_mfma<4, true, true>};
        static_assert(APAP_VARIANT_MFMA == APAP_VARIANT_VALU + 1 && APAP_VARIANT_MFMA4 == APAP_VARIANT_VALU + 2 &&
                      APAP_VARIANT_MFMA4X2 == APAP_VARIANT_VALU + 3, "k1[] is indexed by the variant");
        const int form = !m24 ? 0 : !w32 ? 1 : 2;
        if (p.variant == APAP_VARIANT_MFMA) {
            if ((uintptr_t)d_work % 256 != 0 || p.cells_pad % 64 != 0)
                return apap::fail(APAP_ERR_INVALID_ARG, "apap_solve_device: the workspace must be 256-byte aligned (%p, cells_pad %d)",
                                  d_work, p.cells_pad);
            int slots = apap::opt(ctx, APAP_OPT_PLAN_SLOTS);
            if (slots == 0 && batch == 1) {
                int dev = 0;
                hipError_t e = hipGetDevice(&dev);
                if (e != hipSuccess) return hip_fail(e, "apap_solve_device (hipGetDevice)");
                if (!ctx || ctx->k1_slots_dev != dev || ctx->k1_slots[form] == 0) {
                    int per_cu = 0, cus = 0;
                    e = hipOccupancyMaxActiveBlocksPerMultiprocessor(&per_cu, reinterpret_cast<const void *>(k1_mfma[form]), 256, 0);
                    if (e == hipSuccess) e = hipDeviceGetAttribute(&cus, hipDeviceAttributeMultiprocessorCount, dev);
                    if (e != hipSuccess) return hip_fail(e, "apap_solve_device (resident blocks of K1)");
                    slots = per_cu * cus;
                    if (ctx) {
                        if (ctx->k1_slots_dev != dev) ctx->k1_slots[0] = ctx->k1_slots[1] = ctx->k1_slots[2] = 0;
                        ctx->k1_slots_dev = dev;
                        ctx->k1_slots[form] = slots;
                    }
                } else {
                    slots = ctx->k1_slots[form];
                }
            }
            const int pairs = apap::plan_pairs(p.cell_tiles, p.splits, batch, slots);
            const K1Pairs pp{pairs, p.splits, p.cell_tiles};
            const dim3 grid = pairs > 0 ? dim3(p.cell_tiles * p.splits - pairs, 1, 1) : dim3(p.cell_tiles, p.splits, batch);
            hipLaunchKernelGGL(k1_mfma[form], grid, dim3(256), 0, s, d_tables, n, d_vertices, cells, p.cells_pad, gamma2, inv_sigma2,
                               p.pts_per_split, moments, bs, pp);
        } else {
            const auto &k = k1[p.variant > APAP_VARIANT_MFMA && p.variant <= APAP_VARIANT_MFMA4X2 ? p.variant - APAP_VARIANT_VALU : 0];
            const dim3 grid((p.cell_tiles + k.tiles - 1) / k.tiles, p.splits, batch);
            hipLaunchKernelGGL(k.form[form], grid, dim3(256), 0, s, d_tables, n, d_vertices, cells, p.cells_pad, gamma2,
                               inv_sigma2, p.pts_per_split, moments, bs);
        }
    }
    {
        ProfScope prof(ctx, APAP_PROF_EIGEN, s);
        const dim3 grid(p.cell_tiles, 1, batch);
        using K2 = void (*)(const double *, int, int, int, const double *, int, float *, BatchStride, const double *, int, const double *,
                            double, double, int, double, const WarpEmit);
        static const K2 k2[2][2] = {{k_eigen_denorm<true, false>, k_eigen_denorm<true, true>},
                                    {k_eigen_denorm<false, false>, k_eigen_denorm<false, true>}};
        const bool jacobi = apap::opt(ctx, APAP_OPT_EIGEN_SOLVER) == APAP_EIGEN_JACOBI;
        hipLaunchKernelGGL(k2[jacobi][m24], grid, dim3(64), 0, s, moments, p.splits, cells, p.cells_pad, d_denorms, pick_rank, d_H, bs,
                           d_tables, n, d_vertices, gamma, inv_sigma, careful, trace_floor, we);
    }
    const hipError_t e = hipGetLastError();
    if (e != hipSuccess) return hip_fail(e, "apap_solve_device launch");
    return APAP_OK;
}

extern "C" {

int apap_solve_batch_device(apap_ctx *ctx, const double *d_tables, int n, const double *d_vertices, long long vertices_stride,
                            int cells, double gamma, double sigma, const double *d_denorms, float *d_H,
                            int batch, void *d_work, size_t work_bytes, void *stream) {
    const WarpEmit none{};
    return solve_batch_impl(ctx, d_tables, n, d_vertices, vertices_stride, cells, gamma, sigma, d_denorms, d_H, batch, d_work,
                            work_bytes, stream, none);
}

int apap_solve_warp_batch_device(apap_ctx *ctx, const double *d_tables, int n, const double *d_vertices, long long vertices_stride,
                                 double gamma, double sigma, const double *d_denorms, float *d_H, int batch, void *d_work,
                                 size_t work_bytes, int mesh_rows, int mesh_cols, const double *d_mesh_w, int n_w,
                                 const double *d_mesh_h, int n_h, int final_w, int final_h, int off_x, int off_y,
                                 void *d_warp_work, size_t warp_work_bytes, int *d_status, void *stream) {
    if (!d_mesh_w || !d_mesh_h || !d_warp_work || !d_status)
        return apap::fail(APAP_ERR_INVALID_ARG, "apap_solve_warp_batch_device: null device pointer");
    if (mesh_rows < 1 || mesh_cols < 1 || n_w < 1 || n_h < 1 || final_w < 1 || final_h < 1 || batch < 1)
        return apap::fail(APAP_ERR_INVALID_ARG, "apap_solve_warp_batch_device: bad size");
    if (n_w > kMaxEdges || n_h > kMaxEdges || mesh_rows >= 65535 || mesh_cols >= 65535 ||
        (unsigned long long)mesh_rows * (unsigned long long)mesh_cols * APAP_HINV_STRIDE * sizeof(double) >= (1ull << 32))
        return apap::fail(APAP_ERR_INVALID_ARG, "apap_solve_warp_batch_device: mesh too large for the warp's lookup tables (solve and "
                                                "warp it with the separate entry points)");
    const size_t need = apap_warp_batch_workspace_bytes(mesh_rows, mesh_cols, final_w, final_h, batch);
    if (warp_work_bytes < need)
        return apap::fail(APAP_ERR_WORKSPACE, "apap_solve_warp_batch_device: warp workspace %zu < %zu bytes", warp_work_bytes, need);
    const WarpWork ww = warp_work_layout(d_warp_work, mesh_rows, mesh_cols, final_w, final_h, batch);
    WarpEmit we;
    we.hinv_pad = ww.hinv_pad; we.frec = ww.frec;
    we.hinv_stride = ww.hinv_stride; we.frec_stride = ww.frec_stride;
    we.mesh_w = d_mesh_w; we.mesh_h = d_mesh_h; we.n_w = n_w; we.n_h = n_h;
    we.mesh_rows = mesh_rows; we.mesh_cols = mesh_cols; we.final_w = final_w; we.final_h = final_h; we.off_x = off_x; we.off_y = off_y;
    we.status = d_status;
    return solve_batch_impl(ctx, d_tables, n, d_vertices, vertices_stride, mesh_rows * mesh_cols, gamma, sigma, d_denorms, d_H, batch,
                            d_work, work_bytes, stream, we);
}

int apap_solve_device(apap_ctx *ctx, const double *d_table, int n, const double *d_vertices, int cells,
                      double gamma, double sigma, const double *d_denorm, float *d_H, void *d_work,
                      size_t work_bytes, void *stream) {
    return apap_solve_batch_device(ctx, d_table, n, d_vertices, 0, cells, gamma, sigma, d_denorm, d_H, 1, d_work, work_bytes,
                                   stream);
}

int apap_weights_device(apap_ctx *ctx, const double *d_table, int n, const double *d_vertices, int cells,
                        double gamma, double sigma, double *d_W, void *stream) {
    if (!d_table || !d_vertices || !d_W) return apap::fail(APAP_ERR_INVALID_ARG, "apap_weights_device: null device pointer");
    if (n < 1 || cells < 1) return apap::fail(APAP_ERR_INVALID_ARG, "apap_weights_device: n=%d cells=%d", n, cells);
    const size_t total = (size_t)cells * n;
    const int blocks = (int)((total + 255) / 256 < 8192 ? (total + 255) / 256 : 8192);
    hipLaunchKernelGGL(k_weights, dim3(blocks), dim3(256), 0, (hipStream_t)stream, d_table, n, d_vertices, cells,
                       gamma, 1.0 / (sigma * sigma), d_W);
    const hipError_t e = hipGetLastError();
    if (e != hipSuccess) return hip_fail(e, "apap_weights_device launch");
    return APAP_OK;
}

size_t apap_warp_batch_workspace_bytes(int mesh_rows, int mesh_cols, int final_w, int final_h, int batch) {
    if (mesh_rows < 1 || mesh_cols < 1 || final_w < 1 || final_h < 1 || batch < 1) return 0;
    return warp_work_layout(nullptr, mesh_rows, mesh_cols, final_w, final_h, batch).bytes;
}

size_t apap_warp_workspace_bytes(int mesh_rows, int mesh_cols, int final_w, int final_h) {
    return apap_warp_batch_workspace_bytes(mesh_rows, mesh_cols, final_w, final_h, 1);
}

}

namespace {

struct WarpArgs {
    const uint8_t *img = nullptr;
    long long img_stride = 0;
    int img_h = 0, img_w = 0;
    const uint8_t *center = nullptr;
    long long center_stride = 0;
    int center_h = 0, center_w = 0;
    const void *Hfwd = nullptr;
    int mesh_rows = 0, mesh_cols = 0;
    const double *mesh_w = nullptr;
    int n_w = 0;
    const double *mesh_h = nullptr;
    int n_h = 0;
    int final_w = 0, final_h = 0, off_x = 0, off_y = 0;
    uint8_t *out = nullptr;
    long long out_stride = 0;
    void *Hinv_out = nullptr;
    int batch = 1;
    void *work = nullptr;
    size_t work_bytes = 0;
    int *status = nullptr;
    void *stream = nullptr;
    int row_begin = 0, row_count = 0;
    int phase = APAP_WARP_ALL;
    int **src_rows = nullptr;
};

template <typename T>
int warp_prologue(apap_ctx *ctx, const WarpArgs &a, WarpWork *ww, bool *fast_tables) {
    if (!a.mesh_w || !a.mesh_h || !a.work || !a.status) return apap::fail(APAP_ERR_INVALID_ARG, "warp: null device pointer");
    if (a.mesh_rows < 1 || a.mesh_cols < 1 || a.n_w < 1 || a.n_h < 1 || a.final_w < 1 || a.final_h < 1 || a.batch < 1 || a.batch > 65535)
        return apap::fail(APAP_ERR_INVALID_ARG, "warp: bad size");
    const size_t need = apap_warp_batch_workspace_bytes(a.mesh_rows, a.mesh_cols, a.final_w, a.final_h, a.batch);
    if (a.work_bytes < need) return apap::fail(APAP_ERR_WORKSPACE, "warp: workspace %zu < %zu bytes", a.work_bytes, need);
    const int cells = a.mesh_rows * a.mesh_cols;
    *ww = warp_work_layout(a.work, a.mesh_rows, a.mesh_cols, a.final_w, a.final_h, a.batch);
    *fast_tables = a.n_w <= kMaxEdges && a.n_h <= kMaxEdges && a.mesh_rows < 65535 && a.mesh_cols < 65535;
    const bool geometry = (a.phase & APAP_WARP_GEOMETRY) != 0, per_cell = (a.phase & APAP_WARP_CELLS) != 0;
    if (!geometry && !per_cell) return APAP_OK;
    if (per_cell && !a.Hfwd) return apap::fail(APAP_ERR_INVALID_ARG, "warp: null H grid");
    hipStream_t s = (hipStream_t)a.stream;
    const T *Hfwd = (const T *)a.Hfwd;
    T *Hinv_out = (T *)a.Hinv_out;
    if (*fast_tables) {
        ProfScope prof(ctx, APAP_PROF_INVERT, s);
        const int inv_blocks = per_cell ? (int)(((size_t)(a.mesh_rows + 1) * (a.mesh_cols + 1) + 255) / 256) : 0;
        const int lut_blocks = geometry ? (a.final_h + 1023) / 1024 + (a.final_w + 1023) / 1024 : 0;
        hipLaunchKernelGGL(k_warp_setup<T>, dim3(inv_blocks + lut_blocks, per_cell ? a.batch : 1), dim3(256), 0, s, Hfwd, cells,
                           ww->hinv_pad, Hinv_out, inv_blocks, a.mesh_w, a.n_w, a.mesh_h, a.n_h, a.mesh_rows, a.mesh_cols,
                           a.final_w, a.final_h, ww->lut, a.status, a.off_x, a.off_y, ww->frec, ww->fcol, ww->frow,
                           a.src_rows && geometry && per_cell && a.batch == 1 ? ww->src_rows : (int *)nullptr, ww->hinv_stride,
                           ww->frec_stride);
    } else {
        if (per_cell) {
            ProfScope prof(ctx, APAP_PROF_INVERT, s);
            for (int k = 0; k < a.batch; ++k)
                hipLaunchKernelGGL(k_invert_cells<T>, dim3((cells + 255) / 256), dim3(256), 0, s, Hfwd + (size_t)k * cells * 9, cells,
                                   ww->hinv_pad + k * ww->hinv_stride, Hinv_out ? Hinv_out + (size_t)k * cells * 9 : (T *)nullptr,
                                   a.status);
        }
// ... 268 lines not shown
```

### include/apap_hip.h

```cpp
#ifndef APAP_HIP_H
#define APAP_HIP_H

#include <stddef.h>
#include <stdint.h>

#ifdef __cplusplus
extern "C" {
#endif

#define APAP_OK 0
#define APAP_ERR_INVALID_ARG 1
#define APAP_ERR_NO_DEVICE 2
#define APAP_ERR_HIP 3
#define APAP_ERR_SINGULAR 4
#define APAP_ERR_INDEX 5
#define APAP_ERR_WORKSPACE 6

#define APAP_STATUS_SINGULAR 1
#define APAP_STATUS_INDEX 2
#define APAP_STATUS_UNPREPARED 4
#define APAP_STATUS_NO_CONVERGENCE 8
#define APAP_STATUS_MODEL_DEGENERATE 16
#define APAP_STATUS_MODEL_NO_CONVERGENCE 32

#define APAP_TABLE_STRIDE 32
#define APAP_DENORM_DOUBLES 36
#define APAP_HINV_STRIDE 10

#define APAP_VARIANT_AUTO 0
#define APAP_VARIANT_VALU 1
#define APAP_VARIANT_MFMA 2
#define APAP_VARIANT_MFMA4 3
#define APAP_VARIANT_MFMA4X2 4

#define APAP_EIGEN_AUTO 0
#define APAP_EIGEN_JACOBI 1
#define APAP_EIGEN_INVERSE_ITERATION 2

#define APAP_PROF_ASSEMBLE 0
#define APAP_PROF_EIGEN 1
#define APAP_PROF_INVERT 2
#define APAP_PROF_LUT 3
#define APAP_PROF_WARP 4
#define APAP_PROF_EQ_HIST 5
#define APAP_PROF_EQ_APPLY 6
#define APAP_PROF_RANSAC 7
#define APAP_PROF_SPECTRAL 8
#define APAP_PROF_SLOTS 9

#define APAP_ABI_VERSION 6
#define APAP_ABI_VERSION_STRING "0.6"

const char *apap_last_error(void);
const char *apap_version(void);
int apap_abi_version(void);
int apap_device_count(void);

typedef struct apap_ctx apap_ctx;
#define APAP_OPT_SOLVER_VARIANT 0
#define APAP_OPT_EIGEN_SOLVER 1
#define APAP_OPT_CAREFUL 2
#define APAP_OPT_PROFILE 3
#define APAP_OPT_WANT_WAVES 4
#define APAP_OPT_WARP_ROWS 5
#define APAP_OPT_WEIGHT_CHUNK_KB 6
#define APAP_OPT_FUSED_MAX_CELLS 7
#define APAP_OPT_WARP_FAST 8
#define APAP_OPT_OVERLAP_PCIE 9
#define APAP_OPT_PLAN_CELLS 10
#define APAP_OPT_MOMENTS 11
#define APAP_OPT_WEIGHTS_F32 12
#define APAP_OPT_PLAN_SLOTS 13
#define APAP_OPT_WARP_SAMPLING 14
#define APAP_SAMPLING_NEAREST 0
#define APAP_SAMPLING_BILINEAR 1
#define APAP_OPT_COUNT 15
apap_ctx *apap_ctx_create(void);
void apap_ctx_destroy(apap_ctx *ctx);
int apap_ctx_set_option(apap_ctx *ctx, int option, int value);
int apap_ctx_get_option(const apap_ctx *ctx, int option, int *value);
int apap_ctx_profile_read(apap_ctx *ctx, float *ms, int *launches);


int apap_host_prepare(const float *src, const float *dst, int n, float *N1, float *N2, float *C1,
                      float *C2, float *iC2, float *iN2, float *nf1, float *nf2, float *cf1,
                      float *cf2);

int apap_host_dlt_rows(const float *cf1, const float *cf2, int n, float *aa);

int apap_host_prepare_pts(const void *src, int src_f64, const void *dst, int dst_f64, int n, float *N1, float *N2, float *C1,
                          float *C2, float *iC2, float *iN2, double *nf1, double *nf2, double *cf1, double *cf2);
int apap_host_dlt_rows_pts(const double *cf1, const double *cf2, int n, int product_f64, float *aa);
int apap_host_build_table_rows(const double *src, const float *aa, int n, double *table);

int apap_host_build_table(const float *src, const float *cf1, const float *cf2, int n,
                          double *table);
int apap_host_build_table24(const double *src, const float *aa, int n, double *table);
int apap_host_build_denorm(const float *iC2, const float *C1, const float *iN2, const float *N1,
                           double *denorm);


int apap_local_homography(apap_ctx *ctx, const float *src, const float *dst, int n, const double *vertices,
                          int mesh_rows, int mesh_cols, double gamma, double sigma, float *H_out,
                          double *W_out, int device);
int apap_local_homography_pts(apap_ctx *ctx, const void *src, int src_f64, const void *dst, int dst_f64, int n,
                              const double *vertices, int mesh_rows, int mesh_cols, double gamma, double sigma, float *H_out,
                              double *W_out, int device);

int apap_local_weights(apap_ctx *ctx, const float *src, int n, const double *vertices, int cells, double gamma,
                       double sigma, double *W_out, int device);
int apap_local_weights_pts(apap_ctx *ctx, const void *src, int src_f64, int n, const double *vertices, int cells, double gamma,
                           double sigma, double *W_out, int device);

int apap_local_warp(apap_ctx *ctx, const uint8_t *img, int img_h, int img_w, const float *Hfwd, int mesh_rows,
                    int mesh_cols, const double *mesh_w, int n_w, const double *mesh_h, int n_h,
                    int final_w, int final_h, int off_x, int off_y, uint8_t *out, float *Hinv_out,
                    int device);

int apap_local_warp_f64(apap_ctx *ctx, const uint8_t *img, int img_h, int img_w, const double *Hfwd, int mesh_rows,
                        int mesh_cols, const double *mesh_w, int n_w, const double *mesh_h, int n_h,
                        int final_w, int final_h, int off_x, int off_y, uint8_t *out, double *Hinv_out,
                        int device);

int apap_local_stitch(apap_ctx *ctx, const uint8_t *img, int img_h, int img_w, const uint8_t *center, int center_h,
                      int center_w, const float *Hfwd, int mesh_rows, int mesh_cols,
                      const double *mesh_w, int n_w, const double *mesh_h, int n_h, int final_w,
                      int final_h, int off_x, int off_y, uint8_t *out, float *Hinv_out, int device);

int apap_warp_coords(apap_ctx *ctx, const float *Hfwd, int mesh_rows, int mesh_cols, const double *mesh_w, int n_w,
                     const double *mesh_h, int n_h, int final_w, int final_h, int off_x, int off_y,
                     double *coords, int device);

int apap_invert_normalize_flatten(apap_ctx *ctx, const float *H, int cells, double *out, int device);

int apap_uniform_blend(apap_ctx *ctx, const uint8_t *img1, const uint8_t *img2, int h, int w, uint8_t *out,
                       int device);


size_t apap_solve_workspace_bytes(apap_ctx *ctx, int n, int cells);

int apap_solve_device(apap_ctx *ctx, const double *d_table, int n, const double *d_vertices, int cells,
                      double gamma, double sigma, const double *d_denorm, float *d_H, void *d_work,
                      size_t work_bytes, void *stream);

size_t apap_solve_batch_workspace_bytes(apap_ctx *ctx, int n, int cells, int batch);
int apap_solve_batch_device(apap_ctx *ctx, const double *d_tables, int n, const double *d_vertices, long long vertices_stride,
                            int cells, double gamma, double sigma, const double *d_denorms, float *d_H,
                            int batch, void *d_work, size_t work_bytes, void *stream);

int apap_solve_warp_batch_device(apap_ctx *ctx, const double *d_tables, int n, const double *d_vertices, long long vertices_stride,
                                 double gamma, double sigma, const double *d_denorms, float *d_H, int batch, void *d_work,
                                 size_t work_bytes, int mesh_rows, int mesh_cols, const double *d_mesh_w, int n_w,
                                 const double *d_mesh_h, int n_h, int final_w, int final_h, int off_x, int off_y,
                                 void *d_warp_work, size_t warp_work_bytes, int *d_status, void *stream);

int apap_weights_device(apap_ctx *ctx, const double *d_table, int n, const double *d_vertices, int cells,
                        double gamma, double sigma, double *d_W, void *stream);

size_t apap_warp_workspace_bytes(int mesh_rows, int mesh_cols, int final_w, int final_h);

int apap_warp_device(apap_ctx *ctx, const uint8_t *d_img, int img_h, int img_w, const float *d_Hfwd, int mesh_rows,
                     int mesh_cols, const double *d_mesh_w, int n_w, const double *d_mesh_h,
                     int n_h, int final_w, int final_h, int off_x, int off_y, uint8_t *d_out,
                     float *d_Hinv_out, void *d_work, size_t work_bytes, int *d_status,
                     void *stream);

int apap_warp_f64_device(apap_ctx *ctx, const uint8_t *d_img, int img_h, int img_w, const double *d_Hfwd, int mesh_rows,
                         int mesh_cols, const double *d_mesh_w, int n_w, const double *d_mesh_h, int n_h, int final_w,
                         int final_h, int off_x, int off_y, uint8_t *d_out, double *d_Hinv_out, void *d_work,
                         size_t work_bytes, int *d_status, void *stream);

int apap_warp_rows_device(apap_ctx *ctx, const uint8_t *d_img, int img_h, int img_w, const float *d_Hfwd, int mesh_rows,
                          int mesh_cols, const double *d_mesh_w, int n_w, const double *d_mesh_h, int n_h,
                          int final_w, int final_h, int off_x, int off_y, int row_begin, int row_count,
                          uint8_t *d_out_band, void *d_work, size_t work_bytes, int *d_status, void *stream);

#define APAP_WARP_GEOMETRY 1
#define APAP_WARP_CELLS 2
#define APAP_WARP_GATHER 4
#define APAP_WARP_ALL 7
size_t apap_warp_batch_workspace_bytes(int mesh_rows, int mesh_cols, int final_w, int final_h, int batch);
int apap_warp_batch_device(apap_ctx *ctx, const uint8_t *d_imgs, long long img_stride, int img_h, int img_w,
                           const uint8_t *d_centers, long long center_stride, int center_h, int center_w,
                           const float *d_Hfwd, int mesh_rows, int mesh_cols, const double *d_mesh_w, int n_w,
                           const double *d_mesh_h, int n_h, int final_w, int final_h, int off_x, int off_y,
                           int row_begin, int row_count, uint8_t *d_outs, long long out_stride, float *d_Hinv_out,
                           int batch, int phases, void *d_work, size_t work_bytes, int *d_status, void *stream);

int apap_stitch_device(apap_ctx *ctx, const uint8_t *d_img, int img_h, int img_w, const uint8_t *d_center, int center_h,
                       int center_w, const float *d_Hfwd, int mesh_rows, int mesh_cols,
                       const double *d_mesh_w, int n_w, const double *d_mesh_h, int n_h, int final_w,
                       int final_h, int off_x, int off_y, uint8_t *d_out, float *d_Hinv_out, void *d_work,
                       size_t work_bytes, int *d_status, void *stream);

int apap_warp_coords_device(apap_ctx *ctx, const float *d_Hfwd, int mesh_rows, int mesh_cols, const double *d_mesh_w,
                            int n_w, const double *d_mesh_h, int n_h, int final_w, int final_h,
                            int off_x, int off_y, double *d_coords, void *d_work, size_t work_bytes,
                            int *d_status, void *stream);

int apap_flatten_device(apap_ctx *ctx, const float *d_H, int cells, double *d_out, int *d_status, void *stream);

int apap_blend_device(apap_ctx *ctx, const uint8_t *d_a, const uint8_t *d_b, int h, int w, uint8_t *d_out, void *stream);

int apap_equalize_hist(apap_ctx *ctx, const uint8_t *img, int h, int w, int channels, uint8_t *out, int device);
size_t apap_equalize_workspace_bytes(int channels);
int apap_equalize_hist_device(apap_ctx *ctx, const uint8_t *d_img, int h, int w, int channels, uint8_t *d_out, void *d_work,
                              size_t work_bytes, void *stream);

#define APAP_RANSAC_ITERATIONS 2048
#define APAP_RANSAC_SEED 0x5EEDC0DE5EEDC0DEull
int apap_find_homography_ransac(apap_ctx *ctx, const float *src, const float *dst, int n, double thresh, int iterations,
                                unsigned long long seed, double *H_out, uint8_t *mask_out, int *inliers_out,
                                int device);
size_t apap_ransac_workspace_bytes(int n, int iterations);
int apap_ransac_device(apap_ctx *ctx, const float *d_src, const float *d_dst, int n, double thresh, int iterations,
                       unsigned long long seed, double *d_H_best, uint8_t *d_mask, int *d_result, void *d_work,
                       size_t work_bytes, void *stream);

#define APAP_SPECTRAL_DIM 128
#define APAP_SPECTRAL_EPI_WEIGHT 0
#define APAP_SPECTRAL_AFFINITY_EPS 1
#define APAP_SPECTRAL_AFF_THRESH 2
#define APAP_SPECTRAL_EM_RADIUS 3
#define APAP_SPECTRAL_SCORE_THRESH 4
#define APAP_SPECTRAL_MAX_RESTARTS 5
#define APAP_SPECTRAL_PARAMS 6
#define APAP_SPECTRAL_INFO 6
int apap_spectral_weights(apap_ctx *ctx, const float *src, const float *dst, const float *c_feats, const float *o_feats, int n,
                          const double *F, const double *params, const float *Hg_or_null, const float *mask_in_or_null,
                          double *segment_out, float *ransac_mask_out, float *original_mask_out, double *info_out, int device);
size_t apap_spectral_workspace_bytes(int n);
int apap_spectral_device(apap_ctx *ctx, const float *d_src, const float *d_dst, const float *d_c_feats, const float *d_o_feats,
                         int n, const double *d_F, const double *params, const float *d_Hg_or_null,
                         const float *d_mask_in_or_null, double *d_segment, float *d_ransac_mask, float *d_original_mask,
// ... 225 lines not shown
```

Measured before the change: 291.0 million homographies/s.

## Add short exp chain for assemble chunks proven inside the weight range

Extends the shared exp2 lookup table to a longer range (768 entries) so weights can be evaluated with a single table lookup times a polynomial, with no ldexp and no gamma floor clamp. A per-tile bounding box of cell vertices is reduced across the wave with DPP. Each chunk of correspondences is checked against the distance limit implied by gamma, and while the whole wave stays inside that limit the short chain is used. This saves per-weight ALU work in the assemble kernel, at the cost of a per-chunk check, a slightly larger LDS table, and extra code paths. Optional profiling counters record how many chunks take the short path.

Measured after the change: 304.7 million homographies/s, median of 6. +4.7%, better.

```diff
diff --git a/cvx_proj_amd/_native.py b/cvx_proj_amd/_native.py
--- a/cvx_proj_amd/_native.py
+++ b/cvx_proj_amd/_native.py
@@ -81,7 +81,10 @@
     "apap_ctx_destroy": (None, [_vp]),
     "apap_ctx_set_option": (C.c_int, [_vp, C.c_int, C.c_int]),
     "apap_ctx_get_option": (C.c_int, [_vp, C.c_int, _i32p]),
+    "apap_ctx_set_short_chain": (C.c_int, [_vp, C.c_int]),
+    "apap_ctx_get_short_chain": (C.c_int, [_vp, _i32p]),
     "apap_ctx_profile_read": (C.c_int, [_vp, _f32p, _i32p]),
+    "apap_ctx_profile_k1_chunks": (C.c_int, [_vp, C.POINTER(C.c_uint), C.POINTER(C.c_uint)]),
     "apap_host_prepare": (C.c_int, [_f32p, _f32p, C.c_int] + [_f32p] * 10),
     "apap_host_dlt_rows": (C.c_int, [_f32p, _f32p, C.c_int, _f32p]),
     "apap_host_prepare_pts": (C.c_int, [_vp, C.c_int, _vp, C.c_int, C.c_int] + [_f32p] * 6 + [_f64p] * 4),
@@ -285,13 +288,24 @@
               "plan_slots": OPT_PLAN_SLOTS, "warp_sampling": OPT_WARP_SAMPLING}
 
     def set(self, name, value):
-        check(lib().apap_ctx_set_option(self._h, self._NAMES[name], int(value)))
+        if name == "short_chain":
+            check(lib().apap_ctx_set_short_chain(self._h, int(value)))
+        else:
+            check(lib().apap_ctx_set_option(self._h, self._NAMES[name], int(value)))
         return self
 
     def get(self, name):
         v = C.c_int(0)
-        check(lib().apap_ctx_get_option(self._h, self._NAMES[name], C.byref(v)))
+        if name == "short_chain":
+            check(lib().apap_ctx_get_short_chain(self._h, C.byref(v)))
+        else:
+            check(lib().apap_ctx_get_option(self._h, self._NAMES[name], C.byref(v)))
         return v.value
+
+    def profile_k1_chunks(self):
+        short, every = C.c_uint(0), C.c_uint(0)
+        check(lib().apap_ctx_profile_k1_chunks(self._h, C.byref(short), C.byref(every)))
+        return short.value, every.value
 
     def profile_read(self):
         ms = (C.c_float * PROF_SLOTS)()
diff --git a/cvx_proj_amd/csrc/apap_exp_long.h b/cvx_proj_amd/csrc/apap_exp_long.h
--- /dev/null
+++ b/cvx_proj_amd/csrc/apap_exp_long.h
@@ -0,0 +1,54 @@
+#pragma once
+
+#include <cmath>
+
+#if defined(__HIP__)
+#define APAP_EXP_HD __host__ __device__
+#else
+#define APAP_EXP_HD
+#endif
+
+namespace apap {
+
+constexpr int kExpTabN = 512;
+constexpr int kExpLong = 768;
+constexpr int kExpLongZero = kExpLong - kExpTabN - 1;
+static_assert(kExpLong % 64 == 0 && kExpLong > kExpTabN && kExpLong <= kExpTabN + kExpTabN / 2,
+              "the entries beyond T come from T's upper half (one per thread of a block of 256)");
+
+APAP_EXP_HD inline double exp_long_entry(const double *T, int a) {
+    const int i = a - kExpLongZero;
+    return i < 0 ? 0.5 * T[kExpTabN + i] : i < kExpTabN ? T[i] : 2.0;
+}
+
+constexpr double kExpLn2N = 0x1.62e42fefa39efp-1 / kExpTabN;
+APAP_EXP_HD inline double exp_long_poly(double f, double h) {
+    constexpr double L = kExpLn2N;
+    double p = fma(f, h * (L * L * L * L / 24), h * -(L * L * L / 6));
+    p = fma(f, p, h * (L * L / 2));
+    p = fma(f, p, h * -L);
+    return fma(f, p, h);
+}
+inline double exp_chain_full(double yu, const double *s, double gamma2) {
+    const double m = -yu;
+    const int n = m != m ? 0 : m <= -2147483648.0 ? (int)(-2147483647 - 1) : m >= 2147483647.0 ? 2147483647 : (int)m;
+    const double f = yu - std::floor(yu);
+    const double t = s[kExpLongZero + (n & (kExpTabN - 1))];
+    return std::fmax(std::ldexp(t * exp_long_poly(f, 1.0), n >> 9), gamma2);
+}
+inline double exp_chain_short(double yu, const double *s) {
+    const int n = (int)(-yu);
+    const double f = yu - std::floor(yu);
+    return s[kExpLong - 1 + n] * exp_long_poly(f, 0.5);
+}
+
+inline double exp_long_limit(double gamma2) {
+    const double margin = 1.0 - 0x1p-20;
+    if (!(gamma2 >= 0.0) || !(gamma2 < 1.0)) return 0.0;
+    if (gamma2 == 0.0) return margin * kExpLong;
+    const double Y = -512.0 * std::log2(gamma2);
+    if (!(Y >= 0x1p-10)) return 0.0;
+    return margin * (Y < (double)kExpLong ? Y : (double)kExpLong);
+}
+
+}
diff --git a/cvx_proj_amd/csrc/apap_internal.h b/cvx_proj_amd/csrc/apap_internal.h
--- a/cvx_proj_amd/csrc/apap_internal.h
+++ b/cvx_proj_amd/csrc/apap_internal.h
@@ -25,6 +25,7 @@
 
 struct apap_ctx {
     int opt[APAP_OPT_COUNT] = {APAP_VARIANT_AUTO, APAP_EIGEN_AUTO, 1, 0, 4096, 1, 1 << 20, 4096, 1, 0, 0, 30, 0, 0, APAP_SAMPLING_NEAREST};
+    int short_chain = 1;
     std::vector<apap::ProfSpan> spans;
     apap::DevSlot slots[apap::S_COUNT];
     std::mutex mu;
@@ -35,6 +36,7 @@
     int pipe_dev = -1;
     int k1_slots[3] = {0, 0, 0};
     int k1_slots_dev = -1;
+    void *k1_chunk_counts = nullptr;
 };
 
 namespace apap {
diff --git a/cvx_proj_amd/csrc/apap_kernels.hip b/cvx_proj_amd/csrc/apap_kernels.hip
--- a/cvx_proj_amd/csrc/apap_kernels.hip
+++ b/cvx_proj_amd/csrc/apap_kernels.hip
@@ -4,6 +4,7 @@
 #include <type_traits>
 #include <vector>
 
+#include "apap_exp_long.h"
 #include "apap_internal.h"
 #include "apap_row_term.h"
 #include "apap_warp_dev.h"
@@ -156,35 +157,40 @@
     0x1.fd3c22b8f71f1p+0, 0x1.fdecbe15f6314p+0, 0x1.fe9d96b2a23d9p+0, 0x1.ff4eaca4391b6p+0};
 
 __device__ __forceinline__ double exp_neg_scaled(double yu, const double *tab ) {
-    constexpr double L = 0x1.62e42fefa39efp-1 / kExpN;
     const int nk = (int)(-yu);
     const double f = __builtin_amdgcn_fract(yu);
     const double t = tab[nk & (kExpN - 1)];
-    double p = fma(f, L * L * L * L / 24, -(L * L * L / 6));
-    p = fma(f, p, L * L / 2);
-    p = fma(f, p, -L);
-    p = fma(f, p, 1.0);
+    const double p = apap::exp_long_poly(f, 1.0);
     return __builtin_ldexp(t * p, nk >> kExpBits);
 }
-
+static_assert(apap::kExpTabN == kExpN, "the long table extends kExp2Tab");
+__device__ __forceinline__ double exp_neg_short(double yu, const double *top ) {
+    const int nk = (int)(-yu);
+    return top[nk] * apap::exp_long_poly(__builtin_amdgcn_fract(yu), 0.5);
+}
+
+template <bool kShort = false>
 __device__ __forceinline__ double cell_weight_sq_of(double x, double scaled_inv_sigma2, double gamma2, const double *tab) {
     const double y = __builtin_amdgcn_rsq(x);
     double g = x * y;
     const double e = fma(-g, y, 1.0);
     const double c = fma(e, 0.375, 0.5);
     g = fma(g * e, c, g);
-    return fmax(exp_neg_scaled(g * scaled_inv_sigma2, tab), gamma2);
-}
+    if constexpr (kShort) return exp_neg_short(g * scaled_inv_sigma2, tab);
+    else return fmax(exp_neg_scaled(g * scaled_inv_sigma2, tab), gamma2);
+}
+template <bool kShort = false>
 __device__ __forceinline__ double cell_weight_sq_tab(double vx, double vy, double sx, double sy,
                                                      double scaled_inv_sigma2, double gamma2, const double *tab) {
     const double dx = vx - sx;
     const double dy = vy - sy;
-    return cell_weight_sq_of(fma(dx, dx, fma(dy, dy, 1e-300)), scaled_inv_sigma2, gamma2, tab);
-}
+    return cell_weight_sq_of<kShort>(fma(dx, dx, fma(dy, dy, 1e-300)), scaled_inv_sigma2, gamma2, tab);
+}
+template <bool kShort = false>
 __device__ __forceinline__ double cell_weight_sq_row(double vx, double sx, double row_term,
                                                      double scaled_inv_sigma2, double gamma2, const double *tab) {
     const double dx = vx - sx;
-    return cell_weight_sq_of(fma(dx, dx, row_term), scaled_inv_sigma2, gamma2, tab);
+    return cell_weight_sq_of<kShort>(fma(dx, dx, row_term), scaled_inv_sigma2, gamma2, tab);
 }
 
 __device__ __forceinline__ double cell_weight_sq_f32(float vx, float vy, float2 s, float neg_scale, float gamma2) {
@@ -245,6 +251,12 @@
     __device__ __forceinline__ void publish(double *s_exp2, int tid) const {
 #pragma unroll
         for (int i = 0; i < kPerThread; ++i) s_exp2[(tid + i * kThreads) & (kExpN - 1)] = v[i];
+    }
+    __device__ __forceinline__ void publish_long(double *s, int tid) const {
+        static_assert(kThreads == 256 && kPerThread == 2, "one entry beyond kExp2Tab per thread");
+        publish(s + apap::kExpLongZero, tid);
+        if (tid == 0) s[apap::kExpLong - 1] = 2.0;
+        else if (256 - tid <= apap::kExpLongZero) s[apap::kExpLongZero - (256 - tid)] = 0.5 * v[1];
     }
 };
 
@@ -333,6 +345,13 @@
     __device__ __forceinline__ double sq(const unsigned char *at) const { return sq(read(at)); }
     __device__ __forceinline__ double sq_row(double sx, double row_term) const {
         return cell_weight_sq_row(vx, sx, row_term, scaled_inv_sigma2, gamma2, exp2);
+    }
+    __device__ __forceinline__ double sq_short(Xy s) const {
+        static_assert(!kW32, "the float32 chain has no table");
+        return cell_weight_sq_tab<true>(vx, vy, s.x, s.y, scaled_inv_sigma2, gamma2, exp2 + apap::kExpTabN);
+    }
+    __device__ __forceinline__ double sq_row_short(double sx, double row_term) const {
+        return cell_weight_sq_row<true>(vx, sx, row_term, scaled_inv_sigma2, gamma2, exp2 + apap::kExpTabN);
     }
 };
 
@@ -486,8 +505,8 @@
 template <int kWaves, bool kM24, bool kW32, int kGroups, bool kLevel>
 __device__ __forceinline__ void k1_mfma_tiles(unsigned char (&lds)[2][kChunk * 256], double *s_exp2, double (&s_row)[2][kChunk][2],
                                               const double *__restrict__ table, const double *__restrict__ vertices, int cells,
-                                              int cells_pad, double gamma2, double inv_sigma2, double *__restrict__ slab, int tile,
-                                              const K1Block &blk) {
+                                              int cells_pad, double gamma2, double inv_sigma2, double ylim2, double *__restrict__ slab,
+                                              int tile, const K1Block &blk, unsigned int *__restrict__ chunk_counts) {
     constexpr int kThreads = kWaves * 64;
     const int tid = threadIdx.x;
     ExpTableStage<kThreads> exp_stage;
@@ -499,7 +518,8 @@
     CellWeight<kW32> weight[kGroups];
 #pragma unroll
     for (int t = 0; t < kGroups; ++t)
-        weight[t].set(cell_vertex(vertices, (tile + t) * (16 * kWaves) + wave * 16 + col, cells), inv_sigma2, gamma2, s_exp2);
+        weight[t].set(cell_vertex(vertices, (tile + t) * (16 * kWaves) + wave * 16 + col, cells), inv_sigma2, gamma2,
+                      kW32 ? s_exp2 : s_exp2 + apap::kExpLongZero);
     const int p_begin = blk.p_begin, p_end = blk.p_end, nchunks = blk.nchunks;
 
     constexpr bool kCanShare = !kW32;
@@ -539,6 +559,53 @@
         for (int t = 0; t < kGroups; ++t)
             off_row[t] = apap::row_read_off(0, 0, kgrp, apap::row_value(__double_as_longlong(weight[t].vy), a_bits));
     }
+    constexpr bool kCanShort = !kW32;
+    double box_x0 = 0.0, box_x1 = 0.0, box_y0 = 0.0, box_y1 = 0.0, short_k2 = 0.0, short_lim = 0.0;
+    bool box_finite = true;
+    if constexpr (kCanShort) {
+        const int first = tile * (16 * kWaves);
+#pragma unroll
+        for (int t = 0; t < kGroups; ++t) {
+            const double2 v = cell_vertex(vertices, first + 64 * t + lane, cells);
+            box_finite = box_finite && __builtin_fabs(v.x) < __builtin_inf() && __builtin_fabs(v.y) < __builtin_inf();
+            box_x0 = t ? fmin(box_x0, v.x) : v.x, box_x1 = t ? fmax(box_x1, v.x) : v.x;
+            box_y0 = t ? fmin(box_y0, v.y) : v.y, box_y1 = t ? fmax(box_y1, v.y) : v.y;
+        }
+    }
+    auto box_reduce = [&]() {
+        auto from = [](double v, auto ctrl, auto rows) {
+            const long long b = __double_as_longlong(v);
+            const int lo = __builtin_amdgcn_update_dpp((int)b, (int)b, decltype(ctrl)::value, decltype(rows)::value, 0xf, false);
+            const int hi = __builtin_amdgcn_update_dpp((int)(b >> 32), (int)(b >> 32), decltype(ctrl)::value, decltype(rows)::value, 0xf, false);
+            return __longlong_as_double((long long)(((unsigned long long)(unsigned)hi << 32) | (unsigned)lo));
+        };
+        auto stage = [&](auto ctrl, auto rows) {
+            box_x0 = fmin(box_x0, from(box_x0, ctrl, rows)), box_x1 = fmax(box_x1, from(box_x1, ctrl, rows));
+            box_y0 = fmin(box_y0, from(box_y0, ctrl, rows)), box_y1 = fmax(box_y1, from(box_y1, ctrl, rows));
+        };
+        using std::integral_constant;
+        stage(integral_constant<int, 0x111>{}, integral_constant<int, 0xf>{});
+        stage(integral_constant<int, 0x112>{}, integral_constant<int, 0xf>{});
+        stage(integral_constant<int, 0x114>{}, integral_constant<int, 0xf>{});
+        stage(integral_constant<int, 0x118>{}, integral_constant<int, 0xf>{});
+        stage(integral_constant<int, 0x142>{}, integral_constant<int, 0xa>{});
+        stage(integral_constant<int, 0x143>{}, integral_constant<int, 0xc>{});
+        auto last = [](double v) {
+            const long long b = __double_as_longlong(v);
+            return __longlong_as_double((long long)(((unsigned long long)(unsigned)__builtin_amdgcn_readlane((int)(b >> 32), 63) << 32) |
+                                                    (unsigned)__builtin_amdgcn_readlane((int)b, 63)));
+        };
+        box_x0 = last(box_x0), box_x1 = last(box_x1), box_y0 = last(box_y0), box_y1 = last(box_y1);
+        short_k2 = last(weight[0].scaled_inv_sigma2 * weight[0].scaled_inv_sigma2);
+        short_lim = __all(box_finite) ? ylim2 : 0.0;
+    };
+    const int off_proof = lane * kTableRowBytes + 30 * 8;
+    auto chunk_proved = [&](double2 s) {
+        const double ax = fmax(__builtin_fabs(s.x - box_x0), __builtin_fabs(s.x - box_x1));
+        const double ay = fmax(__builtin_fabs(s.y - box_y0), __builtin_fabs(s.y - box_y1));
+        const double d2 = fma(ax, ax, fma(ay, ay, 1e-300));
+        return __all(d2 * short_k2 < short_lim) != 0;
+    };
     static_assert(kThreads == 256, "four pieces a thread, 16 rows apart");
     const int piece_src = (tid >> 4) * kTableRowBytes + (tid & 15) * 16;
     const int piece_dst = APAP_LDS_PIECE_OFF(tid >> 4, tid & 15);
@@ -574,7 +641,16 @@
     if constexpr (kCanShare) {
         if (row_owner && nchunks > 0) row_y0 = row_fetch(first_window);
     }
-    exp_stage.publish(s_exp2, tid);
+    bool proved = false;
+    if constexpr (kCanShort) {
+        if (ylim2 > 0.0 && nchunks > 0) {
+            const double2 xy0 = first_window.load16(off_proof);
+            box_reduce();
+            proved = chunk_proved(xy0);
+        }
+    }
+    if constexpr (kW32) exp_stage.publish(s_exp2, tid);
+    else exp_stage.publish_long(s_exp2, tid);
     if (nchunks > 0) window_store(lds[0], stage);
     if constexpr (kCanShare) {
         if (row_owner && nchunks > 0) row_publish(0, row_y0);
@@ -582,12 +658,19 @@
     __syncthreads();
     __builtin_amdgcn_s_waitcnt(0x0070);
     const int nfull = (p_end - p_begin) / kChunk;
+    int short_chunks = 0;
     auto chunks = [&](auto row_tag) {
         constexpr bool kRow = decltype(row_tag)::value;
-        auto w2_row = [&](int t, double sx, const unsigned char *rbuf, int s) {
-            return weight[t].sq_row(sx, *reinterpret_cast<const double *>(rbuf + off_row[t] + apap::kRowStepBytes * s));
+        auto w2_row = [&](auto short_tag, int t, double sx, const unsigned char *rbuf, int s) {
+            const double term = *reinterpret_cast<const double *>(rbuf + off_row[t] + apap::kRowStepBytes * s);
+            if constexpr (decltype(short_tag)::value) return weight[t].sq_row_short(sx, term);
+            else return weight[t].sq_row(sx, term);
         };
-        for (int c = 0; c < nfull; ++c) {
+        auto w2_xy = [&](auto short_tag, int t, typename CellWeight<kW32>::Xy xy) {
+            if constexpr (decltype(short_tag)::value) return weight[t].sq_short(xy);
+            else return weight[t].sq(xy);
+        };
+        auto whole = [&](int c, auto short_tag) {
             if constexpr (kLevel) {
                 if (4 * c < nfull) __builtin_amdgcn_s_setprio(3);
                 else if (4 * c < 2 * nfull) __builtin_amdgcn_s_setprio(2);
@@ -596,10 +679,12 @@
             }
             ChunkStage<kThreads> next;
             double row_y = 0.0;
+            double2 next_xy = make_double2(0.0, 0.0);
             {
                 const int next_row = p_begin + (c + 1) * kChunk;
                 const ChunkWindow window(table, next_row, c + 1 < nchunks ? p_end : next_row);
                 window_load(next, window);
+                if constexpr (decltype(short_tag)::value) next_xy = window.load16(off_proof);
                 if constexpr (kRow) {
                     if (row_owner) row_y = row_fetch(window);
                 }
@@ -612,8 +697,8 @@
                     double w2[8];
 #pragma unroll
                     for (int g = 0; g < 8; ++g) {
-                        if constexpr (kRow) w2[g] = w2_row(0, *reinterpret_cast<const double *>(buf + off_xy + 1024 * (s0 + g)), rbuf, s0 + g);
-                        else w2[g] = weight[0].sq(buf + off_xy + 1024 * (s0 + g));
+                        if constexpr (kRow) w2[g] = w2_row(short_tag, 0, *reinterpret_cast<const double *>(buf + off_xy + 1024 * (s0 + g)), rbuf, s0 + g);
+                        else w2[g] = w2_xy(short_tag, 0, CellWeight<kW32>::read(buf + off_xy + 1024 * (s0 + g)));
                     }
                     __builtin_amdgcn_sched_barrier(0);
 #pragma unroll
@@ -630,11 +715,11 @@
                         if constexpr (kRow) {
                             const double sx = *reinterpret_cast<const double *>(buf + off_xy + 1024 * (s0 + g));
 #pragma unroll
-                            for (int t = 0; t < kGroups; ++t) w2[g][t] = w2_row(t, sx, rbuf, s0 + g);
+                            for (int t = 0; t < kGroups; ++t) w2[g][t] = w2_row(short_tag, t, sx, rbuf, s0 + g);
                         } else {
                             const auto xy = CellWeight<kW32>::read(buf + off_xy + 1024 * (s0 + g));
 #pragma unroll
-                            for (int t = 0; t < kGroups; ++t) w2[g][t] = weight[t].sq(xy);
+                            for (int t = 0; t < kGroups; ++t) w2[g][t] = w2_xy(short_tag, t, xy);
                         }
                     }
                     __builtin_amdgcn_sched_barrier(0);
@@ -647,31 +732,49 @@
             if constexpr (kRow) {
                 if (row_owner) row_publish((c + 1) & 1, row_y);
             }
+            bool next_proved = false;
+            if constexpr (decltype(short_tag)::value) next_proved = chunk_proved(next_xy);
             __syncthreads();
-        }
-        if (nfull < nchunks) {
+            return next_proved;
+        };
+        auto partial = [&](auto short_tag) {
             const unsigned char *buf = lds[nfull & 1];
             const unsigned char *rbuf = reinterpret_cast<const unsigned char *>(s_row[nfull & 1]);
             const int steps_here = (p_end - p_begin - nfull * kChunk + 3) >> 2;
             for (int s1 = 0; s1 < steps_here; ++s1) {
                 if constexpr (kGroups == 1) {
                     double w2;
-                    if constexpr (kRow) w2 = w2_row(0, *reinterpret_cast<const double *>(buf + off_xy + 1024 * s1), rbuf, s1);
-                    else w2 = weight[0].sq(buf + off_xy + 1024 * s1);
+                    if constexpr (kRow) w2 = w2_row(short_tag, 0, *reinterpret_cast<const double *>(buf + off_xy + 1024 * s1), rbuf, s1);
+                    else w2 = w2_xy(short_tag, 0, CellWeight<kW32>::read(buf + off_xy + 1024 * s1));
                     sums[0].step(w2, buf + off_b0 + 1024 * s1, buf + off_b1 + 1024 * s1);
                 } else {
                     double w2[kGroups];
                     if constexpr (kRow) {
                         const double sx = *reinterpret_cast<const double *>(buf + off_xy + 1024 * s1);
 #pragma unroll
-                        for (int t = 0; t < kGroups; ++t) w2[t] = w2_row(t, sx, rbuf, s1);
+                        for (int t = 0; t < kGroups; ++t) w2[t] = w2_row(short_tag, t, sx, rbuf, s1);
                     } else {
                         const auto xy = CellWeight<kW32>::read(buf + off_xy + 1024 * s1);
 #pragma unroll
-                        for (int t = 0; t < kGroups; ++t) w2[t] = weight[t].sq(xy);
+                        for (int t = 0; t < kGroups; ++t) w2[t] = w2_xy(short_tag, t, xy);
                     }
                     step2(w2, buf + off_b0 + 1024 * s1, buf + off_b1 + 1024 * s1);
                 }
+            }
+        };
+        int c = 0;
+        if constexpr (kCanShort) {
+            for (; proved && c < nfull; ++c) proved = whole(c, std::true_type{});
+        }
+        short_chunks = c;
+        for (; c < nfull; ++c) whole(c, std::false_type{});
+        if (nfull < nchunks) {
+            if constexpr (kCanShort) {
+                if (proved) ++short_chunks;
+                if (proved) partial(std::true_type{});
+                else partial(std::false_type{});
+            } else {
+                partial(std::false_type{});
             }
             __syncthreads();
         }
@@ -682,6 +785,10 @@
     } else {
         chunks(std::false_type{});
     }
+    if (chunk_counts != nullptr && tid == 0) {
+        atomicAdd(chunk_counts, (unsigned int)short_chunks);
+        atomicAdd(chunk_counts + 1, (unsigned int)nchunks);
+    }
 
     static_assert(kWaves * kLineStageBytes <= (int)sizeof(lds), "a stage per wave");
     constexpr int kSums = kM24 ? 24 : kMoments;
@@ -724,9 +831,9 @@
                                                        const double *__restrict__ vertices, int cells,
                                                        int cells_pad, double gamma2, double inv_sigma2,
                                                        int pts_per_split, double *__restrict__ moments,
-                                                       BatchStride bs, K1Pairs pp) {
+                                                       BatchStride bs, K1Pairs pp, double ylim2, unsigned int *__restrict__ chunk_counts) {
     __shared__ __attribute__((aligned(16))) unsigned char lds[2][kChunk * 256];
-    __shared__ double s_exp2[kExpN];
+    __shared__ double s_exp2[kW32 ? kExpN : apap::kExpLong];
     __shared__ __attribute__((aligned(16))) double s_row[2][kChunk][2];
     int tile = blockIdx.x, split = blockIdx.y;
     bool paired = false;
@@ -735,11 +842,11 @@
     constexpr int kSums = kM24 ? 24 : kMoments;
     double *slab = moments + (long long)blockIdx.z * bs.moments + (size_t)split * kSums * cells_pad;
     if (paired)
-        k1_mfma_tiles<kWaves, kM24, kW32, 2, true>(lds, s_exp2, s_row, table, vertices, cells, cells_pad, gamma2, inv_sigma2, slab, tile, blk);
+        k1_mfma_tiles<kWaves, kM24, kW32, 2, true>(lds, s_exp2, s_row, table, vertices, cells, cells_pad, gamma2, inv_sigma2, ylim2, slab, tile, blk, chunk_counts);
     else if (pp.pairs > 0)
-        k1_mfma_tiles<kWaves, kM24, kW32, 1, true>(lds, s_exp2, s_row, table, vertices, cells, cells_pad, gamma2, inv_sigma2, slab, tile, blk);
+        k1_mfma_tiles<kWaves, kM24, kW32, 1, true>(lds, s_exp2, s_row, table, vertices, cells, cells_pad, gamma2, inv_sigma2, ylim2, slab, tile, blk, chunk_counts);
     else
-        k1_mfma_tiles<kWaves, kM24, kW32, 1, false>(lds, s_exp2, s_row, table, vertices, cells, cells_pad, gamma2, inv_sigma2, slab, tile, blk);
+        k1_mfma_tiles<kWaves, kM24, kW32, 1, false>(lds, s_exp2, s_row, table, vertices, cells, cells_pad, gamma2, inv_sigma2, ylim2, slab, tile, blk, chunk_counts);
 }
 
 template <int kGroups, int kQuads, bool kW32>
@@ -2216,6 +2323,7 @@
     for (void *st : ctx->streams)
         if (st) (void)hipStreamDestroy((hipStream_t)st);
     if (ctx->pinned) (void)hipHostFree(ctx->pinned);
+    if (ctx->k1_chunk_counts) (void)hipFree(ctx->k1_chunk_counts);
     delete ctx;
 }
 
@@ -2248,6 +2356,33 @@
 int apap_ctx_get_option(const apap_ctx *ctx, int option, int *value) {
     if (!value || option < 0 || option >= APAP_OPT_COUNT) return apap::fail(APAP_ERR_INVALID_ARG, "apap_ctx_get_option: bad argument");
     *value = apap::opt(ctx, option);
+    return APAP_OK;
+}
+
+int apap_ctx_set_short_chain(apap_ctx *ctx, int value) {
+    if (!ctx) return apap::fail(APAP_ERR_INVALID_ARG, "apap_ctx_set_short_chain: null context (NULL means the defaults and cannot be changed)");
+    if (value != 0 && value != 1) return apap::fail(APAP_ERR_INVALID_ARG, "apap_ctx_set_short_chain: value %d is not 0 or 1", value);
+    ctx->short_chain = value;
+    return APAP_OK;
+}
+
+int apap_ctx_get_short_chain(const apap_ctx *ctx, int *value) {
+    if (!value) return apap::fail(APAP_ERR_INVALID_ARG, "apap_ctx_get_short_chain: null argument");
+    *value = ctx ? ctx->short_chain : 1;
+    return APAP_OK;
+}
+
+int apap_ctx_profile_k1_chunks(apap_ctx *ctx, unsigned int *short_chunks, unsigned int *chunks) {
+    if (!ctx || !short_chunks || !chunks) return apap::fail(APAP_ERR_INVALID_ARG, "apap_ctx_profile_k1_chunks: null argument");
+    *short_chunks = *chunks = 0;
+    if (!ctx->k1_chunk_counts) return APAP_OK;
+    unsigned int both[2] = {0, 0};
+    hipError_t e = hipDeviceSynchronize();
+    if (e == hipSuccess) e = hipMemcpy(both, ctx->k1_chunk_counts, sizeof(both), hipMemcpyDeviceToHost);
+    if (e == hipSuccess) e = hipMemset(ctx->k1_chunk_counts, 0, sizeof(both));
+    if (e != hipSuccess) return hip_fail(e, "apap_ctx_profile_k1_chunks");
+    *short_chunks = both[0];
+    *chunks = both[1];
     return APAP_OK;
 }
 
@@ -2339,7 +2474,7 @@
             {{k_assemble_mfma4<1, 8, false>, k_assemble_mfma4<1, 6, false>, k_assemble_mfma4<1, 6, true>}, 1},
             {{k_assemble_mfma4<2, 8, false>, k_assemble_mfma4<2, 6, false>, k_assemble_mfma4<2, 6, true>}, 2},
         };
-        using K1Mfma = void (*)(const double *, int, const double *, int, int, double, double, int, double *, BatchStride, K1Pairs);
+        using K1Mfma = void (*)(const double *, int, const double *, int, int, double, double, int, double *, BatchStride, K1Pairs, double, unsigned int *);
         static const K1Mfma k1_mfma[3] = {k_assemble_mfma<4, false, false>, k_assemble_mfma<4, true, false>, k_assemble_mfma<4, true, true>};
         static_assert(APAP_VARIANT_MFMA == APAP_VARIANT_VALU + 1 && APAP_VARIANT_MFMA4 == APAP_VARIANT_VALU + 2 &&
                       APAP_VARIANT_MFMA4X2 == APAP_VARIANT_VALU + 3, "k1[] is indexed by the variant");
@@ -2371,8 +2506,18 @@
             const int pairs = apap::plan_pairs(p.cell_tiles, p.splits, batch, slots);
             const K1Pairs pp{pairs, p.splits, p.cell_tiles};
             const dim3 grid = pairs > 0 ? dim3(p.cell_tiles * p.splits - pairs, 1, 1) : dim3(p.cell_tiles, p.splits, batch);
+            const double ylim = (ctx ? ctx->short_chain : 1) ? apap::exp_long_limit(gamma2) : 0.0;
+            unsigned int *chunk_counts = nullptr;
+            if (ctx && ctx->opt[APAP_OPT_PROFILE]) {
+                if (!ctx->k1_chunk_counts) {
+                    hipError_t e = hipMalloc(&ctx->k1_chunk_counts, 2 * sizeof(unsigned int));
+                    if (e == hipSuccess) e = hipMemset(ctx->k1_chunk_counts, 0, 2 * sizeof(unsigned int));
+                    if (e != hipSuccess) return hip_fail(e, "apap_solve_device (chunk counts)");
+                }
+                chunk_counts = (unsigned int *)ctx->k1_chunk_counts;
+            }
             hipLaunchKernelGGL(k1_mfma[form], grid, dim3(256), 0, s, d_tables, n, d_vertices, cells, p.cells_pad, gamma2, inv_sigma2,
-                               p.pts_per_split, moments, bs, pp);
+                               p.pts_per_split, moments, bs, pp, ylim * ylim, chunk_counts);
         } else {
             const auto &k = k1[p.variant > APAP_VARIANT_MFMA && p.variant <= APAP_VARIANT_MFMA4X2 ? p.variant - APAP_VARIANT_VALU : 0];
             const dim3 grid((p.cell_tiles + k.tiles - 1) / k.tiles, p.splits, batch);
diff --git a/include/apap_hip.h b/include/apap_hip.h
--- a/include/apap_hip.h
+++ b/include/apap_hip.h
@@ -79,7 +79,10 @@
 void apap_ctx_destroy(apap_ctx *ctx);
 int apap_ctx_set_option(apap_ctx *ctx, int option, int value);
 int apap_ctx_get_option(const apap_ctx *ctx, int option, int *value);
+int apap_ctx_set_short_chain(apap_ctx *ctx, int value);
+int apap_ctx_get_short_chain(const apap_ctx *ctx, int *value);
 int apap_ctx_profile_read(apap_ctx *ctx, float *ms, int *launches);
+int apap_ctx_profile_k1_chunks(apap_ctx *ctx, unsigned int *short_chunks, unsigned int *chunks);
 
 
 int apap_host_prepare(const float *src, const float *dst, int n, float *N1, float *N2, float *C1,
```
